# Fierykev/RayTraceBVH

Measured on AMD Instinct MI355X. Metric: Mrays/s primary+1-bounce (BASELINE.json's metric, on its config C5: 3840x2160, the 1/2/4/8-GPU config; the metric's @1080p config C3 is the line c3_1080p); BVH build Mtris/s under build, higher is better.
Workload: dtype f32; 1 GPU; C5: synthetic 10M tris (seed 0x5EED0005, box 100x100x50), 3840x2160, primary+1 bounce; width=3840, height=2160, bounces=1, triangles=10000000, parallelism=single GPU

## Files before the change

include/rtbvh.h:

```cpp
#ifndef RTBVH_H
#define RTBVH_H

#include <stddef.h>
#include <stdint.h>

#ifdef __cplusplus
extern "C" {
#endif

#define RTBVH_ABI_VERSION 8

typedef enum {
    RTBVH_OK = 0,
    RTBVH_ERR_INVALID_ARG = 1,
    RTBVH_ERR_HIP = 2,
    RTBVH_ERR_OOM = 3,
    RTBVH_ERR_NOT_READY = 4,
    RTBVH_ERR_STACK_OVERFLOW = 5,
    RTBVH_ERR_IO = 6,
    RTBVH_ERR_NO_DEVICE = 7,
    RTBVH_ERR_COMM = 8
} rtbvh_status;


// ... 7 lines not shown
    float ambient[4];
    float diffuse[4];
    float specular[4];
    float shininess;
    float optical_density;
    float alpha;
    uint32_t specularb;
    int32_t tex_num;
} rtbvh_material;

typedef struct {
    uint32_t parent, child_l, child_r, code;
    float bb_min[3], bb_max[3];
    uint32_t index;
} rtbvh_node;

typedef struct {
    float intensity;
    float origin[3], direction[3], inv_direction[3];
    float color[4];
} rtbvh_ray_present;

typedef struct {
    uint32_t width, height;
    const uint8_t* rgba8;
} rtbvh_texture;

enum {
    RTBVH_MORTON_CPUTESTS = 0,
    RTBVH_MORTON_HLSL = 1
};
enum {
    RTBVH_DELTA_CLZ64 = 0,
    RTBVH_DELTA_CPUTESTS = 1
};
enum {
    RTBVH_FLAG_TIMING = 1u << 0,
    RTBVH_FLAG_COUNT_VISITS = 1u << 1,
    RTBVH_FLAG_REFRACT_RECORDS = 1u << 2,
    RTBVH_FLAG_SORT_BOUNCE = 1u << 3,
    RTBVH_FLAG_NEAREST_FIRST = 1u << 4,
    RTBVH_FLAG_PACKET_PRIMARY = 1u << 5,
    RTBVH_FLAG_REFILL_BOUNCE = 1u << 6,
    RTBVH_FLAG_WIDE_BVH = 1u << 7,
    RTBVH_FLAG_AUTO_WALK = 1u << 8,
    RTBVH_FLAG_BINNED_PRIMARY = 1u << 9,
    RTBVH_FLAG_CERTIFIED = 1u << 10,
    RTBVH_FLAG_MULTI_KERNEL_BUILD = 1u << 16,
    RTBVH_FLAG_SPLIT_SHIFT = 17,
    RTBVH_FLAG_GRAPH = 1u << 20
};

typedef struct {
    int32_t device;
    uint32_t morton_mode;
    uint32_t delta_mode;
    uint32_t flags;
    float scene_bb_min[3];
    float scene_bb_max[3];
    void* stream;
    uint32_t stack_limit;
    uint32_t reserved;
} rtbvh_config;

typedef struct {
    uint32_t num_tris, num_nodes, width, height;
    uint64_t primary_rays, bounce_rays;
    uint64_t internal_visits[2], leaf_visits[2], hits[2];
    uint64_t textured_hits, stack_overflows;
    uint32_t timed_builds, timed_traces;
    float ms_build, ms_trace;
    float ms_stage[8];
    uint64_t trav_wave_steps, trav_mixed_steps, trav_active_lanes;
    uint64_t trav_max_steps, trav_steps_log2[32];
    uint64_t graph_captures;
    uint32_t walk_flags;
    uint32_t walk_state;
    uint64_t packet_steps[2];
    uint64_t cert_traces, redo_total;
    uint64_t bin_entries[2];
    uint64_t redo_rays[2];
    uint64_t trav_longest;
    uint64_t redo_deferred;
} rtbvh_stats;
typedef struct rtbvh_ctx rtbvh_ctx;

void rtbvh_config_default(rtbvh_config* cfg);
rtbvh_status rtbvh_create(const rtbvh_config* cfg, rtbvh_ctx** out);
void rtbvh_destroy(rtbvh_ctx* ctx);
const char* rtbvh_last_error(const rtbvh_ctx* ctx);
int rtbvh_abi_version(void);
uint32_t rtbvh_stats_size(void);

rtbvh_status rtbvh_set_scene(rtbvh_ctx* ctx, const rtbvh_vertex* verts, uint32_t nverts,
                             const uint32_t* indices, uint32_t nidx, const uint32_t* mat_idx,
                             const rtbvh_material* mats, uint32_t nmats,
                             const rtbvh_texture* textures, uint32_t ntex);
rtbvh_status rtbvh_set_camera(rtbvh_ctx* ctx, const float wvp[16], const float wv[16]);

rtbvh_status rtbvh_build(rtbvh_ctx* ctx);
rtbvh_status rtbvh_build_async(rtbvh_ctx* ctx);
rtbvh_status rtbvh_trace(rtbvh_ctx* ctx, uint32_t width, uint32_t height, uint32_t bounces);
rtbvh_status rtbvh_trace_async(rtbvh_ctx* ctx, uint32_t width, uint32_t height, uint32_t bounces);
rtbvh_status rtbvh_compute_bvh(rtbvh_ctx* ctx, uint32_t width, uint32_t height, uint32_t bounces);
rtbvh_status rtbvh_trace_band_async(rtbvh_ctx* ctx, uint32_t width, uint32_t height, uint32_t bounces,
                                    uint32_t rank, uint32_t nranks, float* dev_out, void* stream);
uint32_t rtbvh_band_rows(uint32_t height, uint32_t rank, uint32_t nranks);
uint32_t rtbvh_deal_bands(uint32_t height, uint32_t rank, uint32_t nranks, uint32_t root_share, uint32_t* bands,
                          uint32_t capacity);
uint32_t rtbvh_deal_rows(uint32_t height, uint32_t rank, uint32_t nranks, uint32_t root_share);
rtbvh_status rtbvh_set_band_deal(rtbvh_ctx* ctx, uint32_t root_share);
rtbvh_status rtbvh_verify_walk(rtbvh_ctx* ctx, uint32_t width, uint32_t height, uint32_t bounces,
                               uint64_t* differing_pixels);
rtbvh_status rtbvh_assemble_bands(rtbvh_ctx* ctx, uint32_t width, uint32_t height, uint32_t nranks,
                                  const float* dev_bands, uint32_t stride_rows, float* dev_frame, void* stream);

#define RTBVH_COMM_ID_BYTES 128
rtbvh_status rtbvh_comm_unique_id(uint8_t id[RTBVH_COMM_ID_BYTES]);
rtbvh_status rtbvh_comm_init(rtbvh_ctx* ctx, uint32_t nranks, uint32_t rank, const uint8_t id[RTBVH_COMM_ID_BYTES],
                             void** comm);
rtbvh_status rtbvh_comm_destroy(void* comm);
rtbvh_status rtbvh_trace_tiles(rtbvh_ctx* ctx, uint32_t width, uint32_t height, uint32_t bounces, uint32_t rank,
                               uint32_t nranks, void* comm);
rtbvh_status rtbvh_synchronize(rtbvh_ctx* ctx);

rtbvh_status rtbvh_update_vertices_async(rtbvh_ctx* ctx, const float* dev_positions, uint32_t pos_stride,
                                         const float* dev_normals, uint32_t nrm_stride,
                                         uint32_t first, uint32_t count, void* stream);
rtbvh_status rtbvh_update_vertices_host(rtbvh_ctx* ctx, const float* positions, uint32_t pos_stride,
                                        const float* normals, uint32_t nrm_stride,
                                        uint32_t first, uint32_t count);
rtbvh_status rtbvh_refit_async(rtbvh_ctx* ctx);
rtbvh_status rtbvh_refit(rtbvh_ctx* ctx);

typedef struct {
    float origin[3];
    float t_max;
    float direction[3];
    uint32_t reserved;
} rtbvh_ray;
typedef struct {
    float t, u, v;
    uint32_t tri;
} rtbvh_hit;
enum {
    RTBVH_QUERY_CLOSEST = 0,
    RTBVH_QUERY_ANY = 1u << 0,
    RTBVH_QUERY_SORT = 1u << 1,
    RTBVH_QUERY_COUNT = 1u << 2,
    RTBVH_QUERY_CERTIFIED = 1u << 8
};
rtbvh_status rtbvh_query_async(rtbvh_ctx* ctx, const rtbvh_ray* dev_rays, uint64_t n, rtbvh_hit* dev_hits,
                               uint32_t mode, void* stream);
rtbvh_status rtbvh_query_host(rtbvh_ctx* ctx, const rtbvh_ray* rays, uint64_t n, rtbvh_hit* hits, uint32_t mode);
rtbvh_status rtbvh_query_counts(rtbvh_ctx* ctx, uint64_t out[4]);
rtbvh_status rtbvh_query_walk_counts(rtbvh_ctx* ctx, uint64_t out[4]);


typedef struct {
    float point[3];
    float max_dist2;
} rtbvh_point;
typedef struct {
    float point[3];
    float dist2;
    float u, v;
// ... 75 lines not shown

typedef struct {
    float v0[3];
    uint32_t reserved0;
    float v1[3];
    uint32_t reserved1;
    float v2[3];
    uint32_t reserved2;
} rtbvh_tri;
enum {
    RTBVH_CROSS_SORT = 1u << 1,
    RTBVH_CROSS_COUNT = 1u << 2,
    RTBVH_CROSS_SIZES = 1u << 4,
    RTBVH_CROSS_FILL = 1u << 5
};
rtbvh_status rtbvh_cross_async(rtbvh_ctx* ctx, const rtbvh_tri* dev_tris, uint64_t n, uint64_t* dev_offsets,
                               uint32_t* dev_ids, uint64_t capacity, uint32_t mode, void* stream);
rtbvh_status rtbvh_cross_host(rtbvh_ctx* ctx, const rtbvh_tri* tris, uint64_t n, uint64_t* offsets, uint32_t* ids,
                              uint64_t capacity, uint32_t mode);
rtbvh_status rtbvh_cross_first_async(rtbvh_ctx* ctx, const rtbvh_tri* dev_tris, uint64_t n, uint32_t* dev_first,
                                     uint32_t mode, void* stream);
rtbvh_status rtbvh_cross_first_host(rtbvh_ctx* ctx, const rtbvh_tri* tris, uint64_t n, uint32_t* first,
                                    uint32_t mode);
rtbvh_status rtbvh_cross_counts(rtbvh_ctx* ctx, uint64_t out[4]);

typedef struct {
    float point_q[3];
    float dist2;
    float point_x[3];
    uint32_t tri;
} rtbvh_clearance;
enum {
    RTBVH_CLEARANCE_SORT = 1u << 1,
    RTBVH_CLEARANCE_COUNT = 1u << 2
};
rtbvh_status rtbvh_clearance_async(rtbvh_ctx* ctx, const rtbvh_tri* dev_tris, uint64_t n, float max_dist2,
                                   rtbvh_clearance* dev_out, uint32_t mode, void* stream);
rtbvh_status rtbvh_clearance_host(rtbvh_ctx* ctx, const rtbvh_tri* tris, uint64_t n, float max_dist2,
                                  rtbvh_clearance* out, uint32_t mode);
rtbvh_status rtbvh_clearance_counts(rtbvh_ctx* ctx, uint64_t out[4]);

typedef struct {
    float lo[3];
    uint32_t reserved0;
    float hi[3];
    uint32_t reserved1;
} rtbvh_box;
enum {
    RTBVH_OVERLAP_SORT = 1u << 1,
    RTBVH_OVERLAP_COUNT = 1u << 2,
    RTBVH_OVERLAP_TRIANGLE = 1u << 3,
    RTBVH_OVERLAP_SIZES = 1u << 4,
    RTBVH_OVERLAP_FILL = 1u << 5
};
rtbvh_status rtbvh_overlap_async(rtbvh_ctx* ctx, const rtbvh_box* dev_boxes, uint64_t n, uint64_t* dev_offsets,
                                 uint32_t* dev_ids, uint64_t capacity, uint32_t mode, void* stream);
rtbvh_status rtbvh_overlap_host(rtbvh_ctx* ctx, const rtbvh_box* boxes, uint64_t n, uint64_t* offsets,
                                uint32_t* ids, uint64_t capacity, uint32_t mode);
rtbvh_status rtbvh_overlap_counts(rtbvh_ctx* ctx, uint64_t out[4]);

typedef struct {
    float point[3]; float dist2;
    float u, v; uint32_t tri;
    uint32_t flags;
} rtbvh_signed;
enum { RTBVH_SIGNED_SORT = 1u << 1, RTBVH_SIGNED_COUNT = 1u << 2,
       RTBVH_SIGNED_VOTE3 = 1u << 3,
       RTBVH_SIGNED_INSIDE_ONLY = 1u << 4
        };
rtbvh_status rtbvh_signed_async(rtbvh_ctx* ctx, const rtbvh_point* dev_points, uint64_t n, rtbvh_signed* dev_out,
                                uint32_t mode, void* stream);
rtbvh_status rtbvh_signed_host(rtbvh_ctx* ctx, const rtbvh_point* points, uint64_t n, rtbvh_signed* out,
                               uint32_t mode);
rtbvh_status rtbvh_signed_counts(rtbvh_ctx* ctx, uint64_t out[4]);

rtbvh_status rtbvh_read_framebuffer(rtbvh_ctx* ctx, float* rgba);
rtbvh_status rtbvh_read_intensity(rtbvh_ctx* ctx, float* intensity);
rtbvh_status rtbvh_present(rtbvh_ctx* ctx, uint8_t* rgba8);
rtbvh_status rtbvh_save_bmp(const char* path, const uint8_t* rgba8, uint32_t width, uint32_t height);
const float* rtbvh_framebuffer_device(rtbvh_ctx* ctx);
rtbvh_status rtbvh_read_bvh(rtbvh_ctx* ctx, rtbvh_node* out, uint32_t capacity);
rtbvh_status rtbvh_read_wide(rtbvh_ctx* ctx, uint32_t* records, uint64_t capacity);
rtbvh_status rtbvh_read_qnodes(rtbvh_ctx* ctx, uint32_t* nodes, uint64_t capacity);
rtbvh_status rtbvh_read_morton(rtbvh_ctx* ctx, uint32_t* codes);
rtbvh_status rtbvh_read_sorted(rtbvh_ctx* ctx, uint32_t* sorted_codes, uint32_t* tri_ids);
rtbvh_status rtbvh_read_rays(rtbvh_ctx* ctx, rtbvh_ray_present* reflect_out, rtbvh_ray_present* refract_out);
rtbvh_status rtbvh_get_stats(rtbvh_ctx* ctx, rtbvh_stats* out);
rtbvh_status rtbvh_reset_stats(rtbvh_ctx* ctx);
rtbvh_status rtbvh_set_flags(rtbvh_ctx* ctx, uint32_t flags);
uint64_t rtbvh_bin_builds(rtbvh_ctx* ctx);
uint32_t rtbvh_bin_sets(rtbvh_ctx* ctx);

rtbvh_status rtbvh_sort_pairs_async(rtbvh_ctx* ctx, uint32_t* keys_in, uint32_t* vals_in,
                                    uint32_t* keys_out, uint32_t* vals_out, uint32_t n,
                                    uint32_t key_bits);
rtbvh_status rtbvh_sort_pairs_host(rtbvh_ctx* ctx, const uint32_t* keys, const uint32_t* vals,
                                   uint32_t* keys_out, uint32_t* vals_out, uint32_t n, uint32_t key_bits);
rtbvh_status rtbvh_build_from_codes(rtbvh_ctx* ctx, const uint32_t* sorted_codes,
                                    const float* leaf_boxes, uint32_t n, rtbvh_node* out);

rtbvh_status rtbvh_texture_load_bmp(const char* path, rtbvh_texture* out);
rtbvh_status rtbvh_texture_load_jpeg(const char* path, rtbvh_texture* out);
rtbvh_status rtbvh_texture_decode_jpeg(const uint8_t* data, size_t size, rtbvh_texture* out);
rtbvh_status rtbvh_texture_load(const char* path, rtbvh_texture* out);
void rtbvh_texture_free(rtbvh_texture* tex);
void rtbvh_srgb_table(float out[256]);
typedef struct rtbvh_scene rtbvh_scene;
rtbvh_status rtbvh_scene_load_obj(const char* path, rtbvh_scene** out);
rtbvh_status rtbvh_scene_synthetic(uint64_t seed, uint32_t ntris, const float half_extent[3],
                                   rtbvh_scene** out);
void rtbvh_scene_free(rtbvh_scene* s);
uint32_t rtbvh_scene_num_vertices(const rtbvh_scene* s);
uint32_t rtbvh_scene_num_indices(const rtbvh_scene* s);
uint32_t rtbvh_scene_num_materials(const rtbvh_scene* s);
uint32_t rtbvh_scene_num_textures(const rtbvh_scene* s);
const rtbvh_vertex* rtbvh_scene_vertices(const rtbvh_scene* s);
const uint32_t* rtbvh_scene_indices(const rtbvh_scene* s);
const uint32_t* rtbvh_scene_mat_indices(const rtbvh_scene* s);
const rtbvh_material* rtbvh_scene_materials(const rtbvh_scene* s);
const char* rtbvh_scene_texture_path(const rtbvh_scene* s, uint32_t k);
rtbvh_status rtbvh_set_scene_obj(rtbvh_ctx* ctx, const rtbvh_scene* s, const rtbvh_texture* textures,
                                 uint32_t ntex);
void rtbvh_camera_reference(uint32_t width, uint32_t height, float wvp[16], float wv[16]);
void rtbvh_camera_look(const float eye[3], uint32_t width, uint32_t height, float wvp[16], float wv[16]);
void rtbvh_camera_orbit(float eye[3], uint32_t key);

#ifdef __cplusplus
}
#endif
#endif
```

raytracebvh_amd/_lib.py:

```python
from __future__ import annotations

import ctypes
import os

import numpy as np

HERE = os.path.dirname(os.path.abspath(__file__))
LIB_PATH = os.environ.get("RTBVH_LIB") or os.path.join(HERE, "librtbvh.so")

OK, ERR_INVALID_ARG, ERR_HIP, ERR_OOM, ERR_NOT_READY, ERR_STACK_OVERFLOW, ERR_IO, ERR_NO_DEVICE = range(8)
MORTON_CPUTESTS, MORTON_HLSL = 0, 1
DELTA_CLZ64, DELTA_CPUTESTS = 0, 1
FLAG_TIMING, FLAG_COUNT_VISITS, FLAG_REFRACT_RECORDS, FLAG_SORT_BOUNCE, FLAG_NEAREST_FIRST = 1, 2, 4, 8, 16
FLAG_PACKET_PRIMARY = 1 << 5
FLAG_REFILL_BOUNCE = 1 << 6
FLAG_WIDE_BVH = 1 << 7
FLAG_BINNED_PRIMARY = 1 << 9
FLAG_CERTIFIED = 1 << 10
FLAG_MULTI_KERNEL_BUILD = 1 << 16
FLAG_AUTO_WALK = 1 << 8
FLAG_SPLIT_SHIFT = 17
FLAG_GRAPH = 1 << 20

EXPORTS = [
    "rtbvh_config_default", "rtbvh_create", "rtbvh_destroy", "rtbvh_last_error", "rtbvh_abi_version", "rtbvh_stats_size",
    "rtbvh_set_scene", "rtbvh_set_camera", "rtbvh_build", "rtbvh_build_async", "rtbvh_trace",
    "rtbvh_trace_async", "rtbvh_compute_bvh", "rtbvh_trace_band_async", "rtbvh_band_rows", "rtbvh_verify_walk",
    "rtbvh_deal_bands", "rtbvh_deal_rows", "rtbvh_set_band_deal",
    "rtbvh_synchronize", "rtbvh_read_framebuffer", "rtbvh_read_intensity", "rtbvh_framebuffer_device",
    "rtbvh_read_bvh", "rtbvh_read_wide", "rtbvh_read_qnodes", "rtbvh_read_morton", "rtbvh_read_sorted", "rtbvh_read_rays", "rtbvh_get_stats",
    "rtbvh_reset_stats", "rtbvh_set_flags", "rtbvh_bin_builds", "rtbvh_bin_sets",
    "rtbvh_sort_pairs_async", "rtbvh_sort_pairs_host", "rtbvh_build_from_codes", "rtbvh_scene_load_obj",
    "rtbvh_scene_synthetic", "rtbvh_scene_free", "rtbvh_scene_num_vertices", "rtbvh_scene_num_indices",
    "rtbvh_scene_num_materials", "rtbvh_scene_num_textures", "rtbvh_scene_vertices", "rtbvh_scene_indices",
    "rtbvh_scene_mat_indices", "rtbvh_scene_materials", "rtbvh_scene_texture_path", "rtbvh_set_scene_obj",
    "rtbvh_camera_reference", "rtbvh_camera_look", "rtbvh_camera_orbit", "rtbvh_texture_load_bmp", "rtbvh_texture_load_jpeg", "rtbvh_texture_decode_jpeg",
    "rtbvh_texture_load", "rtbvh_texture_free", "rtbvh_srgb_table",
    "rtbvh_present", "rtbvh_save_bmp", "rtbvh_assemble_bands", "rtbvh_comm_unique_id", "rtbvh_comm_init",
    "rtbvh_comm_destroy", "rtbvh_trace_tiles",
    "rtbvh_query_async", "rtbvh_query_host", "rtbvh_query_counts", "rtbvh_query_walk_counts",
    "rtbvh_nearest_async", "rtbvh_nearest_host", "rtbvh_nearest_counts",
    "rtbvh_within_async", "rtbvh_within_host", "rtbvh_within_counts",
    "rtbvh_knn_async", "rtbvh_knn_host", "rtbvh_knn_counts",
    "rtbvh_allhits_async", "rtbvh_allhits_host", "rtbvh_allhits_counts",
    "rtbvh_overlap_async", "rtbvh_overlap_host", "rtbvh_overlap_counts",
    "rtbvh_signed_async", "rtbvh_signed_host", "rtbvh_signed_counts",
    "rtbvh_khits_async", "rtbvh_khits_host", "rtbvh_khits_counts",
    "rtbvh_collide_async", "rtbvh_collide_host", "rtbvh_collide_counts",
    "rtbvh_cross_async", "rtbvh_cross_host", "rtbvh_cross_first_async", "rtbvh_cross_first_host", "rtbvh_cross_counts",
    "rtbvh_clearance_async", "rtbvh_clearance_host", "rtbvh_clearance_counts",
    "rtbvh_update_vertices_async", "rtbvh_update_vertices_host", "rtbvh_refit_async", "rtbvh_refit",
]
COMM_ID_BYTES = 128

NODE_DTYPE = np.dtype([("parent", "<u4"), ("child_l", "<u4"), ("child_r", "<u4"), ("code", "<u4"),
                       ("bb_min", "<f4", (3,)), ("bb_max", "<f4", (3,)), ("index", "<u4")])
MATERIAL_DTYPE = np.dtype([("ambient", "<f4", (4,)), ("diffuse", "<f4", (4,)), ("specular", "<f4", (4,)),
                           ("shininess", "<f4"), ("optical_density", "<f4"), ("alpha", "<f4"),
                           ("specularb", "<u4"), ("tex_num", "<i4")])
assert NODE_DTYPE.itemsize == 44 and MATERIAL_DTYPE.itemsize == 68
RAY_DTYPE = np.dtype([("origin", "<f4", (3,)), ("t_max", "<f4"), ("direction", "<f4", (3,)), ("reserved", "<u4")])
HIT_DTYPE = np.dtype([("t", "<f4"), ("u", "<f4"), ("v", "<f4"), ("tri", "<u4")])
assert RAY_DTYPE.itemsize == 32 and HIT_DTYPE.itemsize == 16
QUERY_CLOSEST, QUERY_ANY, QUERY_SORT, QUERY_COUNT = 0, 1, 2, 4
QUERY_CERTIFIED = 1 << 8
POINT_DTYPE = np.dtype([("point", "<f4", (3,)), ("max_dist2", "<f4")])
NEAREST_DTYPE = np.dtype([("point", "<f4", (3,)), ("dist2", "<f4"), ("u", "<f4"), ("v", "<f4"), ("tri", "<u4"),
                          ("reserved", "<u4")])
assert POINT_DTYPE.itemsize == 16 and NEAREST_DTYPE.itemsize == 32
NEAREST_SORT, NEAREST_COUNT = 2, 4
PAIR_DTYPE = np.dtype([("tri", "<u4"), ("dist2", "<f4")])
assert PAIR_DTYPE.itemsize == 8
WITHIN_SORT, WITHIN_COUNT, WITHIN_SIZES, WITHIN_FILL = 2, 4, 16, 32
KNN_SORT, KNN_COUNT = 2, 4
KNN_MAX_K = 32
ALLHITS_SORT, ALLHITS_COUNT, ALLHITS_BY_T, ALLHITS_SIZES, ALLHITS_FILL = 2, 4, 8, 16, 32
BOX_DTYPE = np.dtype([("lo", "<f4", (3,)), ("reserved0", "<u4"), ("hi", "<f4", (3,)), ("reserved1", "<u4")])
assert BOX_DTYPE.itemsize == 32
OVERLAP_SORT, OVERLAP_COUNT, OVERLAP_TRIANGLE, OVERLAP_SIZES, OVERLAP_FILL = 2, 4, 8, 16, 32
SIGNED_DTYPE = np.dtype([("point", "<f4", (3,)), ("dist2", "<f4"), ("u", "<f4"), ("v", "<f4"), ("tri", "<u4"),
                         ("flags", "<u4")])
assert SIGNED_DTYPE.itemsize == 32
SIGNED_SORT, SIGNED_COUNT, SIGNED_VOTE3, SIGNED_INSIDE_ONLY = 2, 4, 8, 16
KHITS_SORT, KHITS_COUNT = 2, 4
KHITS_MAX_K = 16
COLLIDE_COUNT, COLLIDE_TRIANGLE, COLLIDE_SIZES, COLLIDE_FILL, COLLIDE_SYMMETRIC = 4, 8, 16, 32, 64
TRI_DTYPE = np.dtype([("v0", "<f4", (3,)), ("reserved0", "<u4"), ("v1", "<f4", (3,)), ("reserved1", "<u4"),
                      ("v2", "<f4", (3,)), ("reserved2", "<u4")])
assert TRI_DTYPE.itemsize == 48
CROSS_SORT, CROSS_COUNT, CROSS_SIZES, CROSS_FILL = 2, 4, 16, 32
CLEARANCE_DTYPE = np.dtype([("point_q", "<f4", (3,)), ("dist2", "<f4"), ("point_x", "<f4", (3,)), ("tri", "<u4")])
assert CLEARANCE_DTYPE.itemsize == 32
CLEARANCE_SORT, CLEARANCE_COUNT = 2, 4


class Config(ctypes.Structure):
    _fields_ = [("device", ctypes.c_int32), ("morton_mode", ctypes.c_uint32), ("delta_mode", ctypes.c_uint32),
                ("flags", ctypes.c_uint32), ("scene_bb_min", ctypes.c_float * 3),
                ("scene_bb_max", ctypes.c_float * 3), ("stream", ctypes.c_void_p),
                ("stack_limit", ctypes.c_uint32), ("reserved", ctypes.c_uint32)]


class Ray(ctypes.Structure):
    _fields_ = [("origin", ctypes.c_float * 3), ("t_max", ctypes.c_float), ("direction", ctypes.c_float * 3),
                ("reserved", ctypes.c_uint32)]


class Hit(ctypes.Structure):
    _fields_ = [("t", ctypes.c_float), ("u", ctypes.c_float), ("v", ctypes.c_float), ("tri", ctypes.c_uint32)]


class Point(ctypes.Structure):
    _fields_ = [("point", ctypes.c_float * 3), ("max_dist2", ctypes.c_float)]


class Nearest(ctypes.Structure):
    _fields_ = [("point", ctypes.c_float * 3), ("dist2", ctypes.c_float), ("u", ctypes.c_float), ("v", ctypes.c_float),
                ("tri", ctypes.c_uint32), ("reserved", ctypes.c_uint32)]


class Texture(ctypes.Structure):
    _fields_ = [("width", ctypes.c_uint32), ("height", ctypes.c_uint32), ("rgba8", ctypes.c_void_p)]


class Stats(ctypes.Structure):
    _fields_ = [("num_tris", ctypes.c_uint32), ("num_nodes", ctypes.c_uint32), ("width", ctypes.c_uint32),
                ("height", ctypes.c_uint32), ("primary_rays", ctypes.c_uint64), ("bounce_rays", ctypes.c_uint64),
                ("internal_visits", ctypes.c_uint64 * 2), ("leaf_visits", ctypes.c_uint64 * 2),
                ("hits", ctypes.c_uint64 * 2), ("textured_hits", ctypes.c_uint64),
                ("stack_overflows", ctypes.c_uint64), ("timed_builds", ctypes.c_uint32),
                ("timed_traces", ctypes.c_uint32), ("ms_build", ctypes.c_float), ("ms_trace", ctypes.c_float),
                ("ms_stage", ctypes.c_float * 8), ("trav_wave_steps", ctypes.c_uint64),
                ("trav_mixed_steps", ctypes.c_uint64), ("trav_active_lanes", ctypes.c_uint64),
                ("trav_max_steps", ctypes.c_uint64), ("trav_steps_log2", ctypes.c_uint64 * 32),
                ("graph_captures", ctypes.c_uint64), ("walk_flags", ctypes.c_uint32),
                ("walk_state", ctypes.c_uint32), ("packet_steps", ctypes.c_uint64 * 2),
                ("cert_traces", ctypes.c_uint64), ("redo_total", ctypes.c_uint64),
                ("bin_entries", ctypes.c_uint64 * 2), ("redo_rays", ctypes.c_uint64 * 2),
                ("trav_longest", ctypes.c_uint64), ("redo_deferred", ctypes.c_uint64)]

    def as_dict(self) -> dict:
        d = {}
        for k, _ in self._fields_:
            v = getattr(self, k)
            d[k] = list(v) if hasattr(v, "__len__") else v
        return d


class RtbvhError(RuntimeError):
    def __init__(self, status: int, msg: str):
        super().__init__(f"rtbvh status {status}: {msg}")
        self.status = status


_lib = None


def lib() -> ctypes.CDLL:
    global _lib
    if _lib is not None:
        return _lib
    if not os.path.exists(LIB_PATH):
        raise ImportError(f"{LIB_PATH} is not built: run `python -c 'import __graft_entry__ as g; g.build()'` "
                          "(there is no CPU fallback for the HIP path)")
    try:
        import torch
    except ImportError:
        pass
    L = ctypes.CDLL(LIB_PATH)
    vp, u32, u64, i32 = ctypes.c_void_p, ctypes.c_uint32, ctypes.c_uint64, ctypes.c_int
    sig = {
        "rtbvh_config_default": (None, [ctypes.POINTER(Config)]),
        "rtbvh_create": (i32, [ctypes.POINTER(Config), ctypes.POINTER(vp)]),
        "rtbvh_destroy": (None, [vp]),
        "rtbvh_last_error": (ctypes.c_char_p, [vp]),
        "rtbvh_abi_version": (i32, []),
        "rtbvh_stats_size": (ctypes.c_uint32, []),
        "rtbvh_set_scene": (i32, [vp, vp, u32, vp, u32, vp, vp, u32, vp, u32]),
        "rtbvh_set_camera": (i32, [vp, vp, vp]),
        "rtbvh_build": (i32, [vp]),
        "rtbvh_build_async": (i32, [vp]),
        "rtbvh_trace": (i32, [vp, u32, u32, u32]),
        "rtbvh_trace_async": (i32, [vp, u32, u32, u32]),
        "rtbvh_compute_bvh": (i32, [vp, u32, u32, u32]),
        "rtbvh_trace_band_async": (i32, [vp, u32, u32, u32, u32, u32, vp, vp]),
        "rtbvh_band_rows": (u32, [u32, u32, u32]),
        "rtbvh_deal_bands": (u32, [u32, u32, u32, u32, vp, u32]),
        "rtbvh_deal_rows": (u32, [u32, u32, u32, u32]),
        "rtbvh_set_band_deal": (i32, [vp, u32]),
        "rtbvh_verify_walk": (i32, [vp, u32, u32, u32, ctypes.POINTER(u64)]),
        "rtbvh_assemble_bands": (i32, [vp, u32, u32, u32, vp, u32, vp, vp]),
        "rtbvh_comm_unique_id": (i32, [vp]),
        "rtbvh_comm_init": (i32, [vp, u32, u32, vp, ctypes.POINTER(vp)]),
        "rtbvh_comm_destroy": (i32, [vp]),
        "rtbvh_trace_tiles": (i32, [vp, u32, u32, u32, u32, u32, vp]),
        "rtbvh_synchronize": (i32, [vp]),
        "rtbvh_read_framebuffer": (i32, [vp, vp]),
        "rtbvh_read_intensity": (i32, [vp, vp]),
        "rtbvh_framebuffer_device": (vp, [vp]),
        "rtbvh_read_bvh": (i32, [vp, vp, u32]),
        "rtbvh_read_morton": (i32, [vp, vp]),
        "rtbvh_read_wide": (i32, [vp, vp, ctypes.c_uint64]),
        "rtbvh_read_qnodes": (i32, [vp, vp, ctypes.c_uint64]),
        "rtbvh_read_sorted": (i32, [vp, vp, vp]),
        "rtbvh_read_rays": (i32, [vp, vp, vp]),
        "rtbvh_get_stats": (i32, [vp, ctypes.POINTER(Stats)]),
        "rtbvh_reset_stats": (i32, [vp]),
        "rtbvh_set_flags": (i32, [vp, u32]),
        "rtbvh_bin_builds": (u64, [vp]),
        "rtbvh_bin_sets": (u32, [vp]),
        "rtbvh_sort_pairs_async": (i32, [vp, vp, vp, vp, vp, u32, u32]),
        "rtbvh_sort_pairs_host": (i32, [vp, vp, vp, vp, vp, u32, u32]),
        "rtbvh_build_from_codes": (i32, [vp, vp, vp, u32, vp]),
        "rtbvh_scene_load_obj": (i32, [ctypes.c_char_p, ctypes.POINTER(vp)]),
        "rtbvh_scene_synthetic": (i32, [u64, u32, vp, ctypes.POINTER(vp)]),
        "rtbvh_scene_free": (None, [vp]),
        "rtbvh_scene_num_vertices": (u32, [vp]),
        "rtbvh_scene_num_indices": (u32, [vp]),
        "rtbvh_scene_num_materials": (u32, [vp]),
        "rtbvh_scene_num_textures": (u32, [vp]),
        "rtbvh_scene_vertices": (vp, [vp]),
        "rtbvh_scene_indices": (vp, [vp]),
        "rtbvh_scene_mat_indices": (vp, [vp]),
        "rtbvh_scene_materials": (vp, [vp]),
        "rtbvh_scene_texture_path": (ctypes.c_char_p, [vp, u32]),
        "rtbvh_set_scene_obj": (i32, [vp, vp, vp, u32]),
        "rtbvh_camera_reference": (None, [u32, u32, vp, vp]),
        "rtbvh_camera_look": (None, [vp, u32, u32, vp, vp]),
        "rtbvh_camera_orbit": (None, [vp, u32]),
        "rtbvh_texture_load_bmp": (i32, [ctypes.c_char_p, vp]),
        "rtbvh_texture_load_jpeg": (i32, [ctypes.c_char_p, vp]),
        "rtbvh_texture_decode_jpeg": (i32, [vp, ctypes.c_size_t, vp]),
        "rtbvh_texture_load": (i32, [ctypes.c_char_p, vp]),
        "rtbvh_texture_free": (None, [vp]),
        "rtbvh_srgb_table": (None, [vp]),
        "rtbvh_present": (i32, [vp, vp]),
        "rtbvh_save_bmp": (i32, [ctypes.c_char_p, vp, u32, u32]),
        "rtbvh_query_async": (i32, [vp, vp, u64, vp, u32, vp]),
        "rtbvh_query_host": (i32, [vp, vp, u64, vp, u32]),
        "rtbvh_query_counts": (i32, [vp, vp]),
        "rtbvh_query_walk_counts": (i32, [vp, vp]),
        "rtbvh_nearest_async": (i32, [vp, vp, u64, vp, u32, vp]),
        "rtbvh_nearest_host": (i32, [vp, vp, u64, vp, u32]),
        "rtbvh_nearest_counts": (i32, [vp, vp]),
        "rtbvh_within_async": (i32, [vp, vp, u64, vp, vp, u64, u32, vp]),
        "rtbvh_within_host": (i32, [vp, vp, u64, vp, vp, u64, u32]),
        "rtbvh_within_counts": (i32, [vp, vp]),
        "rtbvh_knn_async": (i32, [vp, vp, u64, u32, vp, u32, vp]),
        "rtbvh_knn_host": (i32, [vp, vp, u64, u32, vp, u32]),
        "rtbvh_knn_counts": (i32, [vp, vp]),
        "rtbvh_signed_async": (i32, [vp, vp, u64, vp, u32, vp]),
        "rtbvh_signed_host": (i32, [vp, vp, u64, vp, u32]),
        "rtbvh_signed_counts": (i32, [vp, vp]),
        "rtbvh_khits_async": (i32, [vp, vp, u64, u32, vp, u32, vp]),
        "rtbvh_khits_host": (i32, [vp, vp, u64, u32, vp, u32]),
        "rtbvh_khits_counts": (i32, [vp, vp]),
        "rtbvh_allhits_async": (i32, [vp, vp, u64, vp, vp, u64, u32, vp]),
        "rtbvh_allhits_host": (i32, [vp, vp, u64, vp, vp, u64, u32]),
        "rtbvh_allhits_counts": (i32, [vp, vp]),
        "rtbvh_overlap_async": (i32, [vp, vp, u64, vp, vp, u64, u32, vp]),
        "rtbvh_overlap_host": (i32, [vp, vp, u64, vp, vp, u64, u32]),
        "rtbvh_overlap_counts": (i32, [vp, vp]),
        "rtbvh_collide_async": (i32, [vp, vp, vp, u64, u32, vp]),
        "rtbvh_collide_host": (i32, [vp, vp, vp, u64, u32]),
        "rtbvh_collide_counts": (i32, [vp, vp]),
        "rtbvh_cross_async": (i32, [vp, vp, u64, vp, vp, u64, u32, vp]),
        "rtbvh_cross_host": (i32, [vp, vp, u64, vp, vp, u64, u32]),
        "rtbvh_cross_first_async": (i32, [vp, vp, u64, vp, u32, vp]),
        "rtbvh_cross_first_host": (i32, [vp, vp, u64, vp, u32]),
        "rtbvh_cross_counts": (i32, [vp, vp]),
        "rtbvh_clearance_async": (i32, [vp, vp, u64, ctypes.c_float, vp, u32, vp]),
        "rtbvh_clearance_host": (i32, [vp, vp, u64, ctypes.c_float, vp, u32]),
        "rtbvh_clearance_counts": (i32, [vp, vp]),
        "rtbvh_update_vertices_async": (i32, [vp, vp, u32, vp, u32, u32, u32, vp]),
        "rtbvh_update_vertices_host": (i32, [vp, vp, u32, vp, u32, u32, u32]),
        "rtbvh_refit_async": (i32, [vp]),
        "rtbvh_refit": (i32, [vp]),
    }
    for name, (res, args) in sig.items():
        f = getattr(L, name)
        f.restype = res
        f.argtypes = args
    _lib = L
    return L


# ... 12 lines not shown
```

raytracebvh_amd/csrc/api.hip:

```cpp
#include <dlfcn.h>
#include <rccl/rccl.h>

#include <algorithm>
#include <cstdio>
#include <cstring>
#include <deque>
#include <new>
#include <string>
#include <type_traits>
#include <utility>
#include <vector>

#include "../../include/rtbvh.h"
#include "rtbvh_internal.h"

using namespace rtbvh;

#ifndef RTBVH_MAXSPLIT
#define RTBVH_MAXSPLIT 4
#endif

template <typename H, void (*Del)(H)>
struct Owner {
    H h{};
    Owner() = default;
    Owner(Owner&& o) noexcept : h(o.h) { o.h = H{}; }
    Owner& operator=(Owner&& o) noexcept {
        std::swap(h, o.h);
        return *this;
    }
    ~Owner() { reset(); }
    void reset() {
        if (h) Del(h);
        h = H{};
    }
    H* out() {
        reset();
        return &h;
    }
    operator H() const { return h; }
};
template <typename T> void del_device(T* p) { (void)hipFree((void*)p); }
template <typename T> void del_pinned(T* p) { (void)hipHostFree((void*)p); }
inline void del_event(hipEvent_t e) { (void)hipEventDestroy(e); }
inline void del_stream(hipStream_t s) {
    (void)hipStreamSynchronize(s);
    (void)hipStreamDestroy(s);
}
template <typename T>
struct DevBuf : Owner<T*, del_device<T>> {
    hipError_t alloc(size_t count) { return hipMalloc((void**)this->out(), (count ? count : 1) * sizeof(T)); }
};
template <typename T>
struct Pinned : Owner<T*, del_pinned<T>> {
    hipError_t alloc(size_t count) {
        return hipHostMalloc((void**)this->out(), count * sizeof(T), hipHostMallocDefault);
    }
};
using Event = Owner<hipEvent_t, del_event>;
using Stream = Owner<hipStream_t, del_stream>;
template <typename T>
struct Grown {
    DevBuf<T> buf;
    size_t cap = 0;
    bool has(size_t n) const { return n == 0 || (n <= cap && buf); }
    hipError_t reserve(size_t n) {
        if (has(n)) return hipSuccess;
        const hipError_t e = buf.alloc(n);
        if (e != hipSuccess) buf.h = nullptr;
        cap = e == hipSuccess ? n : 0;
        return e;
    }
    void reset() {
        buf.reset();
        cap = 0;
    }
    operator T*() const { return buf.h; }
};

enum Form : uint32_t { RECORDS = 1, NBOX = 2, PSEUDO = 4, QNODES = 8 };
struct Tree {
    bool built = false;
    bool clz64 = false;
    Form wrote = RECORDS;
    uint32_t valid = 0;
};

struct PbKey {
    uint64_t build = 0;
    uint32_t W = 0, H = 0, rows = 0, rank = 0, nranks = 0, T = 0, ntx = 0, nty = 0;
    uint32_t share = 0;
    const uint32_t* deal = nullptr;
    bool operator==(const PbKey& o) const {
        return build == o.build && W == o.W && H == o.H && rows == o.rows && rank == o.rank &&
               nranks == o.nranks && T == o.T && ntx == o.ntx && nty == o.nty && share == o.share &&
               deal == o.deal;
    }
};
struct PbBufs {
    DevBuf<uint32_t> off, cur, sums;
    DevBuf<uint4> bins;
    uint32_t cap_T = 0, cap_tiles = 0, cap_bins = 0;
    Grown<uint32_t> list;
    PbKey key;
    bool valid = false;
    Event filled;
    uint32_t readers = 0;
};

struct TraceSet {
    Stream chain;
    Event join;
    hipStream_t caller = nullptr;
    Event done;
    bool busy = false;
    DevBuf<RayQ> q[2];
    DevBuf<float2> hit;
    Grown<uint32_t> redo, defer;
    PbBufs pb;
    Grown<unsigned long long> pbkeys;
    uint32_t* qcount = nullptr;
    uint32_t* next = nullptr;
    unsigned long long* counters = nullptr;
    unsigned long long* ovf = nullptr;
};

struct LastTrace {
    bool traced = false;
    uint32_t W = 0, H = 0, bounces = 0, rank = 0, nranks = 1;
    uint32_t nsplit = 1;
    uint32_t slot = 0;
    size_t rec_P = 0;
    uint32_t walk = 0;
    uint32_t walk_state = 0;
    bool cert = false;
    bool frame_here = false;
    bool intensity_here = false;
};

struct rtbvh_ctx {
    rtbvh_config cfg{};
    Stream own_stream, side;
    static constexpr uint32_t MAXSPLIT = RTBVH_MAXSPLIT;
    TraceSet sets[MAXSPLIT];
    hipStream_t stream = nullptr;
    std::string err;

    uint32_t V = 0, T = 0, nmat = 0;
    DevBuf<float4> d_opos;
    DevBuf<float> d_verts;
    DevBuf<uint32_t> d_idx, d_matidx;
    DevBuf<Mat> d_mats;
    float wvp[16], wv[16];
    DevBuf<float> d_cam;
    bool cam_dirty = false;
    bool have_scene = false, have_camera = false;
    Tree tree;
    Event ev_update;
    bool update_pending = false;
    bool stale = false;

    uint32_t cap_T = 0;
    DevBuf<uint32_t> d_codes, d_ids, d_ka, d_va, d_kb, d_vb, d_sort_scratch;
    DevBuf<float4> d_tclip, d_leaf;
    Grown<float4> d_band;
    DevBuf<Inner> d_inner;
    DevBuf<uint4> d_topo;
    DevBuf<Inner> d_rec;
    DevBuf<QNode> d_qnode;
    DevBuf<uint4> d_lfp;
    DevBuf<uint32_t> d_texels;
    DevBuf<uint4> d_texinfo;
    DevBuf<float> d_srgb;
    uint32_t ntex = 0;
    Grown<float> d_refl_rec;
    Grown<float> d_refr_rec;
    DevBuf<uint32_t> d_pleaf, d_pint, d_cnt;
    DevBuf<uint32_t> d_xlist, d_xcnt;
    DevBuf<uint32_t> d_qlate;
    DevBuf<unsigned long long> d_ovf;
    Pinned<unsigned long long> h_ovf;
    unsigned long long ovf_seen = 0;
    DevBuf<float> d_bounds, d_rootbox, d_zpart;
    Event ev_leaf, ev_prim;
    DevBuf<float> d_nbox;
    bool tail_pending = false;
    bool leaf_pending = false;
    SortResult sorted{nullptr, nullptr};

    size_t cap_P = 0;
    DevBuf<float4> d_color;
    DevBuf<float> d_intensity;
    DevBuf<uint32_t> d_bkin, d_bvin, d_bka, d_bva, d_bkb, d_bvb, d_bscratch;
    DevBuf<uint32_t> d_qcount;
    DevBuf<uint32_t> d_next;
    DevBuf<unsigned long long> d_counters;
    size_t cap_split = 0;
    Event ev_fork;
    uint64_t bins_epoch = 1;
    uint64_t bin_builds = 0;
    bool knob_bins_reuse = true;
    LastTrace last;

    static constexpr int RING = 32;
    Event evb[RING][6];
    Event evt[RING][5];
    bool evt_trav[RING] = {};
    uint32_t n_builds = 0, n_traces = 0;
    Event ev_built;
    bool slots_used = false;
    hipGraph_t graph = nullptr;
    hipGraphExec_t graph_exec = nullptr;
    uint64_t graph_key[5] = {};
    bool capturing = false;
    uint64_t graph_captures = 0;
    LastTrace graph_trace;
    Tree graph_tree;
    uint64_t cert_traces = 0;
    uint64_t small_key = 0;
    uint32_t small_flags = 0;
    bool small_packet = false;
    Event ev_small[2];
    uint32_t knob_bounce_blocks = 0;
    bool knob_overlap = false, knob_side_priority = true, knob_keep_records = false, knob_no_early_shade = false,
         knob_no_small_tiles = false;
    uint32_t root_share = 16;
    struct DealTab {
        uint32_t H, nranks, share;
        DevBuf<uint32_t> d;
        std::vector<uint32_t> off;
        Pinned<uint32_t> h;
        Event ready;
    };
    std::deque<DealTab> deals;
    static constexpr size_t MAX_DEALS = 8;
    DevBuf<uint32_t> d_qscratch;
    Grown<uint32_t> d_qsort;
    Grown<uint32_t> d_qsort_scratch;
    Grown<uint32_t> d_qredo;
    Grown<unsigned long long> d_qscan;
    Grown<uint32_t> d_qorder;
    Event ev_query;
    bool query_busy = false;
    bool query_ovf = false;
    bool query_counted = false;
    uint64_t query_fallback = 0;
    bool nearest_counted = false;
    bool within_counted = false;
    bool allhits_counted = false;
    bool overlap_counted = false;
    bool knn_counted = false;
    bool signed_counted = false;
    bool khits_counted = false;
    bool collide_counted = false;
    bool cross_counted = false;
    bool clearance_counted = false;
};

namespace {

std::string g_create_error;

rtbvh_status fail(rtbvh_ctx* c, rtbvh_status st, const std::string& msg) {
    if (c) c->err = msg;
    else g_create_error = msg;
    return st;
}

#define HIPC(ctx, expr)                                                                          \
    do {                                                                                         \
        hipError_t _e = (expr);                                                                  \
        if (_e != hipSuccess)                                                                    \
            return fail(ctx, _e == hipErrorOutOfMemory ? RTBVH_ERR_OOM : RTBVH_ERR_HIP,          \
                        std::string(#expr) + ": " + hipGetErrorString(_e));                      \
    } while (0)
#define TRY(expr)                                      \
    do {                                               \
        if (rtbvh_status _st = (expr)) return _st;     \
    } while (0)

void drop_graph(rtbvh_ctx* c) {
    if (c->graph_exec) (void)hipGraphExecDestroy(c->graph_exec);
    if (c->graph) (void)hipGraphDestroy(c->graph);
    c->graph_exec = nullptr;
    c->graph = nullptr;
}

void reset_tree(rtbvh_ctx* c) {
    c->tree = Tree{};
    c->stale = false;
    c->bins_epoch++;
    c->tail_pending = c->leaf_pending = false;
}

rtbvh_status check_launch(rtbvh_ctx* c, const char* what) {
    hipError_t e = hipGetLastError();
    if (e != hipSuccess) return fail(c, RTBVH_ERR_HIP, std::string(what) + ": " + hipGetErrorString(e));
    return RTBVH_OK;
}

rtbvh_status drain_slots(rtbvh_ctx* c) {
    for (TraceSet& t : c->sets)
        if (t.busy) HIPC(c, hipEventSynchronize(t.done));
    return RTBVH_OK;
}
rtbvh_status sync_all(rtbvh_ctx* c) {
    HIPC(c, hipStreamSynchronize(c->stream));
    TRY(drain_slots(c));
    if (c->query_busy) HIPC(c, hipEventSynchronize(c->ev_query));
    if (c->update_pending) HIPC(c, hipEventSynchronize(c->ev_update));
    return RTBVH_OK;
}

rtbvh_status wait_slots(rtbvh_ctx* c, hipStream_t s) {
    for (TraceSet& t : c->sets)
        if (t.busy) {
            HIPC(c, hipStreamWaitEvent(s, t.done, 0));
            t.busy = false;
        }
    return RTBVH_OK;
}

rtbvh_status wait_queries(rtbvh_ctx* c, hipStream_t s) {
    if (c->query_busy) {
        HIPC(c, hipStreamWaitEvent(s, c->ev_query, 0));
        c->query_busy = false;
    }
    return RTBVH_OK;
}

rtbvh_status wait_update(rtbvh_ctx* c, hipStream_t s) {
    if (c->update_pending) {
        HIPC(c, hipStreamWaitEvent(s, c->ev_update, 0));
        c->update_pending = false;
    }
    return RTBVH_OK;
}
rtbvh_status fail_stale(rtbvh_ctx* c, const char* what) {
    return fail(c, RTBVH_ERR_NOT_READY,
                std::string(what) + ": the vertices were updated after the last build -- the tree is not of this "
                                    "geometry until rtbvh_build, rtbvh_refit or rtbvh_compute_bvh");
}

rtbvh_status order_after_context(rtbvh_ctx* c, hipStream_t s) {
    if (!c->capturing) HIPC(c, hipEventRecord(c->ev_built, c->stream));
    if (s != c->stream) HIPC(c, hipStreamWaitEvent(s, c->ev_built, 0));
    return RTBVH_OK;
}

rtbvh_status ensure_build_capacity(rtbvh_ctx* c, uint32_t T) {
    if (T <= c->cap_T && c->d_codes) return RTBVH_OK;
    drop_graph(c);
    reset_tree(c);
    const size_t n = T, ni = T > 1 ? T - 1 : 1;
    HIPC(c, c->d_codes.alloc(n));
    HIPC(c, c->d_ids.alloc(n));
    HIPC(c, c->d_ka.alloc(n));
    HIPC(c, c->d_va.alloc(n));
    HIPC(c, c->d_kb.alloc(n));
    HIPC(c, c->d_vb.alloc(n));
    HIPC(c, c->d_sort_scratch.alloc(sort_scratch_words(T)));
    HIPC(c, c->d_tclip.alloc(TCS * n));
    HIPC(c, c->d_leaf.alloc(4 * n));
    HIPC(c, c->d_inner.alloc(ni));
    HIPC(c, c->d_topo.alloc(ni));
    HIPC(c, c->d_rec.alloc(2 * (size_t)n - 1));
    HIPC(c, c->d_nbox.alloc(6 * (size_t)ni));
    HIPC(c, c->d_qnode.alloc(2 * (size_t)n - 1));
    HIPC(c, c->d_lfp.alloc(n));
    HIPC(c, c->d_pleaf.alloc(n));
    HIPC(c, c->d_pint.alloc(ni));
    HIPC(c, c->d_cnt.alloc(ni));
    HIPC(c, c->d_xlist.alloc(n));
    HIPC(c, c->d_qlate.alloc(n + 1));
    HIPC(c, c->d_xcnt.alloc(refit_blocks(T)));
    HIPC(c, c->d_zpart.alloc(ZPART * (size_t)refit_blocks(T)));
    HIPC(c, c->d_bounds.alloc(BOUNDS_WORDS));
    HIPC(c, c->d_rootbox.alloc(ROOTBOX_WORDS));
    c->cap_T = T;
    return RTBVH_OK;
}

rtbvh_status ensure_trace_capacity(rtbvh_ctx* c, size_t P) {
    if (P <= c->cap_P && c->d_color) return RTBVH_OK;
    drop_graph(c);
    HIPC(c, c->d_color.alloc(P));
    HIPC(c, c->d_intensity.alloc(P));
    HIPC(c, c->sets[0].q[0].alloc(P));
    HIPC(c, c->sets[0].q[1].alloc(P));
    HIPC(c, c->d_bkin.alloc(P));
    HIPC(c, c->d_bvin.alloc(P));
    HIPC(c, c->d_bka.alloc(P));
    HIPC(c, c->d_bva.alloc(P));
    HIPC(c, c->d_bkb.alloc(P));
    HIPC(c, c->d_bvb.alloc(P));
    HIPC(c, c->d_bscratch.alloc(sort_scratch_words((uint32_t)P)));
    HIPC(c, c->sets[0].hit.alloc(P));
    if (!c->d_qcount) HIPC(c, c->d_qcount.alloc(32 * rtbvh_ctx::MAXSPLIT));
    if (!c->d_next) HIPC(c, c->d_next.alloc((size_t)NEXT_WORDS * rtbvh_ctx::MAXSPLIT));
    if (!c->d_counters) HIPC(c, c->d_counters.alloc(64 * rtbvh_ctx::MAXSPLIT));
    for (uint32_t b = 0; b < rtbvh_ctx::MAXSPLIT; b++) {
        c->sets[b].qcount = c->d_qcount + 32 * b;
        c->sets[b].next = c->d_next + (size_t)NEXT_WORDS * b;
        c->sets[b].counters = c->d_counters + 64 * b;
    }
    c->cap_P = P;
    return RTBVH_OK;
}

uint32_t trace_split(const rtbvh_ctx* c) {
    const uint32_t v = (c->cfg.flags >> RTBVH_FLAG_SPLIT_SHIFT) & 7u;
    if (v) return v < rtbvh_ctx::MAXSPLIT ? v : rtbvh_ctx::MAXSPLIT;
    return 1;
}

rtbvh_status ensure_split_capacity(rtbvh_ctx* c, uint32_t nsets, size_t rays) {
    if (nsets < 2) return RTBVH_OK;
    const bool grow = rays > c->cap_split;
    if (grow) {
        drop_graph(c);
        TRY(drain_slots(c));
        c->cap_split = rays;
        for (uint32_t g = nsets; g < rtbvh_ctx::MAXSPLIT; g++) {
            TraceSet& t = c->sets[g];
            t.q[0].reset(); t.q[1].reset(); t.hit.reset();
        }
    }
    for (uint32_t g = 1; g < nsets; g++) {
        TraceSet& t = c->sets[g];
        if (!t.chain) HIPC(c, hipStreamCreateWithFlags(t.chain.out(), hipStreamNonBlocking));
        if (!t.join) HIPC(c, hipEventCreateWithFlags(t.join.out(), hipEventDisableTiming));
        if (!c->ev_fork) HIPC(c, hipEventCreateWithFlags(c->ev_fork.out(), hipEventDisableTiming));
        if (t.q[0] && !grow) continue;
        HIPC(c, t.q[0].alloc(c->cap_split));
        HIPC(c, t.q[1].alloc(c->cap_split));
        HIPC(c, t.hit.alloc(c->cap_split));
// ... 248 lines not shown
    std::string err;
    ncclResult_t (*GetUniqueId)(ncclUniqueId*) = nullptr;
    ncclResult_t (*CommInitRank)(ncclComm_t*, int, ncclUniqueId, int) = nullptr;
    ncclResult_t (*CommDestroy)(ncclComm_t) = nullptr;
    ncclResult_t (*Send)(const void*, size_t, ncclDataType_t, int, ncclComm_t, hipStream_t) = nullptr;
    ncclResult_t (*Recv)(void*, size_t, ncclDataType_t, int, ncclComm_t, hipStream_t) = nullptr;
    ncclResult_t (*GroupStart)() = nullptr;
    ncclResult_t (*GroupEnd)() = nullptr;
    const char* (*GetErrorString)(ncclResult_t) = nullptr;
};
const Rccl& rccl() {
    static const Rccl lib = [] {
        Rccl r;
        void* h = dlopen("librccl.so.1", RTLD_NOW | RTLD_GLOBAL);
        if (!h) {
            const char* e = dlerror();
            r.err = std::string("RCCL not available: ") + (e ? e : "dlopen(librccl.so.1) failed");
            return r;
        }
        bool all = true;
        auto sym = [&](auto& f, const char* name) {
            f = reinterpret_cast<std::remove_reference_t<decltype(f)>>(dlsym(h, name));
            if (!f) all = false;
        };
        sym(r.GetUniqueId, "ncclGetUniqueId");
        sym(r.CommInitRank, "ncclCommInitRank");
        sym(r.CommDestroy, "ncclCommDestroy");
        sym(r.Send, "ncclSend");
        sym(r.Recv, "ncclRecv");
        sym(r.GroupStart, "ncclGroupStart");
        sym(r.GroupEnd, "ncclGroupEnd");
        sym(r.GetErrorString, "ncclGetErrorString");
        r.ok = all;
        if (!all) r.err = "RCCL: librccl.so.1 lacks a required symbol";
        return r;
    }();
    return lib;
}

rtbvh_status sync_camera(rtbvh_ctx* c, hipStream_t s) {
    if (!c->cam_dirty) return RTBVH_OK;
    TRY(wait_slots(c, c->stream));
    launch_set_camera(c->wvp, c->wv, c->d_cam, c->stream);
    HIPC(c, hipGetLastError());
    c->cam_dirty = false;
    return order_after_context(c, s);
}

rtbvh_status before_tree_write(rtbvh_ctx* c, hipStream_t s) {
    TRY(wait_slots(c, s));
    TRY(wait_queries(c, s));
    TRY(wait_update(c, s));
    TRY(sync_camera(c, s));
    c->bins_epoch++;
    return RTBVH_OK;
}

struct TailGuard {
    rtbvh_ctx* c;
    bool pending;
    void run() {
        if (pending) launch_refit_tail(build_args(c), c->stream);
        pending = false;
    }
    ~TailGuard() { run(); }
};

struct WalkPlan {
    hipStream_t s;
    uint32_t slot, bounces;
    bool cert;
    bool leaf_pending;
    bool count, timing, records;
    Walks wk;
    PrimaryKind pkind;
    Form nodes;
    uint32_t P, rows;
    uint32_t nsplit, Pg;
    uint32_t tblocks;
    uint32_t ntx, nty;
    bool inflight, fuse_tail, overlap, small_tiles, early_shade;
    uint32_t bset;
    bool fill_bins;
};

WalkPlan plan_walks(const rtbvh_ctx* c, const TraceArgs& a, uint32_t bounces, hipStream_t s, uint32_t slot,
                    uint32_t flags, bool cert, bool timed, bool tail_pending, bool leaf_pending) {
    WalkPlan p{s, slot, bounces, cert, leaf_pending};
    p.bset = slot;
    p.count = (c->cfg.flags & RTBVH_FLAG_COUNT_VISITS) != 0;
    p.timing = timed && (c->cfg.flags & RTBVH_FLAG_TIMING) != 0 && s == c->stream && !c->capturing;
    p.wk = choose_walks(flags);
    p.records = (flags & RTBVH_FLAG_REFRACT_RECORDS) != 0;
    p.P = a.W * deal_rows(a.H, a.rank, a.nranks, c->root_share);
    p.rows = p.P / a.W;
#ifndef RTBVH_BOUNCE_GRID
#define RTBVH_BOUNCE_GRID (256 * BOUNCE_WAVES)
#endif
    p.inflight = slot != 0;
    for (uint32_t k = 1; k < rtbvh_ctx::MAXSPLIT && !p.inflight && !c->capturing; k++)
        p.inflight = c->sets[k].busy && hipEventQuery(c->sets[k].done) == hipErrorNotReady;
    p.tblocks = p.P < (1u << 22) ? (!p.inflight ? 1536 : p.P < (3u << 20) ? 512 : 1024) : RTBVH_BOUNCE_GRID;
    if (c->knob_bounce_blocks) p.tblocks = c->knob_bounce_blocks;
    const bool binned = p.wk.primary == PrimaryKind::BINNED;
    p.pkind = binned && (a.W > 32768u || a.H > 32768u)
                  ? (cert ? PrimaryKind::LANE_REFERENCE : PrimaryKind::PACKET_WIDE)
                  : p.wk.primary;
    p.nsplit = trace_split(c);
    if (p.wk.sort || a.my_bands < p.nsplit || slot || c->slots_used || binned) p.nsplit = 1;
    p.Pg = p.nsplit == 1 ? p.P : a.W * 8 * ((a.my_bands + p.nsplit - 1) / p.nsplit);
    p.nodes = cert ? NBOX : RECORDS;
    p.fuse_tail = tail_pending && p.pkind == PrimaryKind::BINNED && s == c->stream && slot == 0 && p.rows > 0 &&
                  (c->tree.valid & p.nodes);
    p.overlap = p.pkind == PrimaryKind::BINNED && leaf_pending && s == c->stream && slot == 0 && p.nsplit == 1;
    p.ntx = pb_tiles_x(a.W);
    p.nty = pb_tiles_y(p.rows);
    p.small_tiles = !p.inflight && !c->knob_no_small_tiles && (size_t)a.W * p.rows < (3u << 19);
    p.early_shade = cert && !p.inflight && !c->knob_no_early_shade;
    return p;
}

rtbvh_status prepare_walks(rtbvh_ctx* c, WalkPlan& p, TraceArgs& a, const rtbvh_ctx::DealTab* deal, TailGuard& tail) {
    hipStream_t s = p.s;
    TraceSet& mine = c->sets[p.slot];
    const size_t P = p.P;
    if (p.records) {
        if (!(c->d_refl_rec.has(14 * P) && c->d_refr_rec.has(14 * P))) {
            drop_graph(c);
            HIPC(c, c->d_refl_rec.reserve(14 * P));
            HIPC(c, c->d_refr_rec.reserve(14 * P));
        }
        a.refl_rec = c->d_refl_rec;
        a.refr_rec = c->d_refr_rec;
    }
    if (!p.fuse_tail && tail.pending) {
        tail.run();
        TRY(order_after_context(c, s));
    }
    TRY(ensure_form(c, p.nodes, s));
    a.nb = p.cert;
    TRY(ensure_split_capacity(c, p.slot ? p.slot + 1 : p.nsplit, p.Pg));
    if (p.bounces > 0 && p.wk.refill && p.wk.bounce == BounceWalk::WIDE_QUANTIZED) TRY(ensure_form(c, QNODES, s));
    if (p.pkind == PrimaryKind::PACKET_REFERENCE || p.pkind == PrimaryKind::PACKET_NEAREST ||
        p.pkind == PrimaryKind::PACKET_WIDE)
        TRY(ensure_form(c, PSEUDO, s));
    if (p.cert && p.bounces > 0 && !mine.defer.has(P)) {
        drop_graph(c);
        HIPC(c, mine.defer.reserve(P));
        if (hipMemsetAsync(mine.defer, 0, sizeof(uint32_t) * P, c->stream) != hipSuccess) {
            mine.defer.reset();
            return fail(c, RTBVH_ERR_HIP, "clearing the deferred-ray list failed");
        }
        TRY(order_after_context(c, s));
    }
    if (p.cert && !mine.redo.has(P)) {
        drop_graph(c);
        HIPC(c, mine.redo.reserve(P));
    }
    if (p.pkind != PrimaryKind::BINNED || p.rows == 0) return RTBVH_OK;
    const size_t px = (size_t)a.W * p.rows;
    if (pb_keys_used() && !mine.pbkeys.has(px)) {
        drop_graph(c);
        HIPC(c, mine.pbkeys.reserve(px));
    }
    const PbKey key{c->bins_epoch, a.W, a.H, p.rows, a.rank, a.nranks, c->T, p.ntx, p.nty,
                    a.nranks > 1 ? c->root_share : 16u, deal ? deal->d.h : nullptr};
    const int found = p.fuse_tail || p.leaf_pending ? -1 : find_bins(c, key);
    if (found >= 0) {
        p.bset = (uint32_t)found;
        PbBufs& pb = c->sets[p.bset].pb;
        if (p.bset != p.slot) HIPC(c, hipStreamWaitEvent(s, pb.filled, 0));
        pb.readers |= 1u << p.slot;
        return RTBVH_OK;
    }
    p.fill_bins = true;
    PbBufs& pb = mine.pb;
    TRY(ensure_pb_capacity(c, pb, c->T, p.ntx * p.nty));
    if (a.nranks > 1 && !pb.list.has(pb_list_words(c->T))) {
        drop_graph(c);
        HIPC(c, pb.list.reserve(pb_list_words(c->T)));
    }
    for (uint32_t k = 0; k < rtbvh_ctx::MAXSPLIT && !c->capturing; k++) {
        if (k == p.slot || !(pb.readers & 1u << k)) continue;
        if (k == 0) TRY(order_after_context(c, s));
        else if (c->sets[k].done) HIPC(c, hipStreamWaitEvent(s, c->sets[k].done, 0));
    }
    pb.readers = 1u << p.slot;
    pb.valid = false;
    pb.key = key;
    return RTBVH_OK;
}

rtbvh_status launch_walks(rtbvh_ctx* c, const WalkPlan& p, const TraceArgs& a, TailGuard& tail) {
    hipStream_t s = p.s;
    TraceSet& mine = c->sets[p.slot];
    const uint32_t bounces = p.bounces, nsplit = p.nsplit;
    const bool count = p.count, cert = p.cert, refill = p.wk.refill;
    Event* ev = c->evt[c->n_traces % rtbvh_ctx::RING];
    ZeroList z{};
    z.ptr[0] = reinterpret_cast<uint32_t*>(mine.counters);
    z.words[0] = 64 * 2;
    z.ptr[1] = mine.qcount;
    z.words[1] = 32 * nsplit;
    if (refill && bounces) {
        z.ptr[2] = mine.next;
        z.words[2] = (size_t)NEXT_WORDS * nsplit;
    }
    if (p.fill_bins) {
        z.ptr[3] = mine.pb.off;
        z.words[3] = (size_t)p.ntx * p.nty * PB_NZ + 1;
        if (a.nranks > 1) {
            z.ptr[4] = mine.pb.list;
            z.words[4] = (size_t)PB_LISTS * PB_LIST_STRIDE;
        }
    }
    hipStream_t sp = s;
    if (p.overlap) {
        sp = c->side;
        HIPC(c, hipStreamWaitEvent(sp, c->ev_leaf, 0));
    }
    launch_zero(z, sp);
    if (p.timing) HIPC(c, hipEventRecord(ev[0], sp));
    if (nsplit > 1) HIPC(c, hipEventRecord(c->ev_fork, s));
    for (uint32_t g = 0; g < nsplit; g++) {
        TraceSet& set = c->sets[p.slot + g];
// ... 17 lines not shown
                    c->bin_builds++;
                    if (c->knob_bins_reuse && !c->capturing) {
                        if (!pbb.filled) HIPC(c, hipEventCreateWithFlags(pbb.filled.out(), hipEventDisableTiming));
                        HIPC(c, hipEventRecord(pbb.filled, sp));
                        pbb.valid = true;
                    }
                }
                launch_pb_raster(ag, pb, p.rows, q[0], &qc[0], count, bounces > 0, sp, cert ? &rd : nullptr,
                                 p.small_tiles);
                if (p.fuse_tail) tail.pending = false;
            }
            if (p.overlap) {
                HIPC(c, hipEventRecord(c->ev_prim, sp));
                HIPC(c, hipStreamWaitEvent(sg, c->ev_prim, 0));
            }
            if (p.rows) launch_pb_gate(ag, pb, q[0], &qc[0], count, bounces > 0, sg, cert);
        } else
            launch_primary(ag, q[0], &qc[0], count, bounces > 0, p.pkind, sg);
        if (tg) HIPC(c, hipEventRecord(ev[1], sg));
        for (uint32_t b = 0; b < bounces; b++) {
            const uint32_t* perm = nullptr;
            if (p.wk.sort) {
                launch_bounce_keys(q[b & 1], &qc[b], c->d_rootbox, p.P, c->d_bkin, c->d_bvin, sg);
                perm = radix_sort_pairs(c->d_bkin, c->d_bvin, c->d_bka, c->d_bva, c->d_bkb, c->d_bvb, p.P, 30,
                                        c->d_bscratch, sg).vals;
            }
            if (refill) {
                if (tg && b == 0) HIPC(c, hipEventRecord(ev[3], sg));
                uint32_t* nxb = set.next + (size_t)NEXT_SEGS * NEXT_STRIDE * b;
                const BounceShade es{q[(b + 1) & 1], &qc[b + 1], b + 1 < bounces, mine.redo, &qc[17 + b], p.Pg};
                launch_bounce_traverse(ag, q[b & 1], &qc[b], perm, count, p.wk.bounce, set.hit, nxb, p.tblocks, sg, cert,
                                       mine.defer, p.early_shade ? &es : nullptr);
                if (tg && b == 0) HIPC(c, hipEventRecord(ev[4], sg));
                const Redo rd{mine.redo, &qc[17 + b], mine.defer, nxb};
                launch_bounce_shade(ag, q[b & 1], &qc[b], set.hit, q[(b + 1) & 1], &qc[b + 1], count, b + 1 < bounces,
                                    p.Pg, sg, cert ? &rd : nullptr);
            } else
                launch_bounce(ag, q[b & 1], &qc[b], perm, q[(b + 1) & 1], &qc[b + 1], count, b + 1 < bounces,
                              p.wk.nearest, sg);
        }
        if (g) {
            HIPC(c, hipEventRecord(set.join, sg));
            HIPC(c, hipStreamWaitEvent(s, set.join, 0));
        }
    }
    HIPC(c, hipMemcpyAsync(mine.ovf, c->d_ovf, sizeof(unsigned long long), hipMemcpyDeviceToHost, s));
    if (p.timing) {
        HIPC(c, hipEventRecord(ev[2], s));
        c->evt_trav[c->n_traces % rtbvh_ctx::RING] = refill && bounces > 0;
        c->n_traces++;
    }
    return RTBVH_OK;
}

rtbvh_status enqueue_walks(rtbvh_ctx* c, uint32_t W, uint32_t H, uint32_t bounces, uint32_t rank, uint32_t nranks,
                           float4* color, float* inten, hipStream_t s, uint32_t slot, uint32_t flags, bool timed,
                           uint32_t walk_state, bool cert = false) {
    const bool leaf_pending = c->leaf_pending;
    c->leaf_pending = false;
    TailGuard tail{c, c->tail_pending};
    c->tail_pending = false;
    if (!c->tree.built) return fail(c, RTBVH_ERR_NOT_READY, "trace before build");
    if (c->stale) return fail_stale(c, "trace");
    if (W == 0 || H == 0 || nranks == 0 || rank >= nranks || bounces > 14)
        return fail(c, RTBVH_ERR_INVALID_ARG, "bad trace dimensions");
    TRY(ensure_trace_capacity(c, (size_t)W * H));
    if (!color) color = c->d_color;
    TraceArgs a = trace_args(c, W, H, rank, nranks, color, inten);
    const rtbvh_ctx::DealTab* deal = nullptr;
    TRY(get_deal(c, H, nranks, &deal, s));
    if (deal) {
        a.my_bands = deal->off[rank + 1] - deal->off[rank];
        a.band_list = deal->d + deal->off[rank];
        a.band_slots = deal->d + (H + 7) / 8;
    }
    a.counters = c->sets[slot].counters;
    if ((flags & RTBVH_FLAG_REFRACT_RECORDS) && slot)
        return fail(c, RTBVH_ERR_INVALID_ARG, "ray records are traced on the context stream only");
    WalkPlan p = plan_walks(c, a, bounces, s, slot, flags, cert, timed, tail.pending, leaf_pending);
    TRY(prepare_walks(c, p, a, deal, tail));
    TRY(launch_walks(c, p, a, tail));
    const bool frame_here = color == c->d_color && nranks == 1;
    c->last = LastTrace{true, W, H, bounces, rank, nranks, p.nsplit, slot, p.records ? p.P : 0, flags & WALK_FLAGS,
                        walk_state, cert, frame_here, frame_here && inten != nullptr};
    return check_launch(c, "trace kernels");
}

struct TracePlan {
    uint32_t flags;
    bool cert;
    uint32_t state;
};
TracePlan plan_trace(const rtbvh_ctx* c, uint32_t f) {
    if (!(f & (RTBVH_FLAG_AUTO_WALK | RTBVH_FLAG_CERTIFIED))) return TracePlan{f, false, 0};
    const uint32_t ref = f & ~WALK_FLAGS;
    const bool limited = c->cfg.stack_limit != 0 && c->cfg.stack_limit < (uint32_t)STACK_SIZE;
    const bool want = (f & RTBVH_FLAG_CERTIFIED) || auto_checked(c);
    if (!want || !c->tree.clz64 || limited) return TracePlan{ref, false, 0};
    return TracePlan{ref | RTBVH_FLAG_NEAREST_FIRST | RTBVH_FLAG_REFILL_BOUNCE | RTBVH_FLAG_WIDE_BVH |
                         RTBVH_FLAG_BINNED_PRIMARY,
                     true, 2};
}

rtbvh_status enqueue_trace(rtbvh_ctx* c, uint32_t W, uint32_t H, uint32_t bounces, uint32_t rank, uint32_t nranks,
                           float4* color, float* inten, hipStream_t s, uint32_t slot = 0) {
    if (!c->tree.built) return fail(c, RTBVH_ERR_NOT_READY, "trace before build");
    if (c->stale) return fail_stale(c, "trace");
    TRY(sync_camera(c, s));
    TracePlan p = plan_trace(c, c->cfg.flags);
    if (p.cert && !c->capturing) c->cert_traces++;
    const uint32_t f = c->cfg.flags;
    const bool limited = c->cfg.stack_limit != 0 && c->cfg.stack_limit < (uint32_t)STACK_SIZE;
    if ((f & RTBVH_FLAG_AUTO_WALK) && !p.cert && c->tree.clz64 && !limited) {
        const uint64_t key = (uint64_t)W << 48 | (uint64_t)H << 32 | c->T;
        const uint32_t fw = f & (WALK_FLAGS | RTBVH_FLAG_AUTO_WALK | RTBVH_FLAG_CERTIFIED | RTBVH_FLAG_SORT_BOUNCE);
        if ((c->small_key != key || c->small_flags != fw) && !c->capturing && s == c->stream && slot == 0 &&
            nranks == 1) {
            Event* ev = c->ev_small;
            for (int k = 0; k < 2; k++)
                if (!ev[k]) HIPC(c, hipEventCreate(ev[k].out()));
            float best[2] = {INFINITY, INFINITY};
            for (int round = 0; round < 2; round++)
                for (int k = 0; k < 2; k++) {
                    HIPC(c, hipEventRecord(ev[0], s));
                    TRY(enqueue_walks(c, W, H, 0, 0, 1, color, inten, s, 0,
                                      p.flags | (k ? RTBVH_FLAG_PACKET_PRIMARY : 0u), false, p.state));
                    HIPC(c, hipEventRecord(ev[1], s));
                    HIPC(c, hipEventSynchronize(ev[1]));
                    float ms = 0.f;
                    HIPC(c, hipEventElapsedTime(&ms, ev[0], ev[1]));
                    best[k] = std::min(best[k], ms);
                }
            c->small_packet = best[1] < 0.95f * best[0];
            c->small_key = key;
            c->small_flags = fw;
        }
        if (c->small_key == key && c->small_flags == fw && c->small_packet) p.flags |= RTBVH_FLAG_PACKET_PRIMARY;
    }
    return enqueue_walks(c, W, H, bounces, rank, nranks, color, inten, s, slot, p.flags, true, p.state, p.cert);
}

}

extern "C" {

int rtbvh_abi_version(void) { return RTBVH_ABI_VERSION; }
uint32_t rtbvh_stats_size(void) { return (uint32_t)sizeof(rtbvh_stats); }

void rtbvh_config_default(rtbvh_config* cfg) {
    if (!cfg) return;
    memset(cfg, 0, sizeof(*cfg));
    cfg->device = 0;
    cfg->morton_mode = RTBVH_MORTON_CPUTESTS;
    cfg->delta_mode = RTBVH_DELTA_CLZ64;
    for (int k = 0; k < 3; k++) {
        cfg->scene_bb_min[k] = -700.f;
        cfg->scene_bb_max[k] = 700.f;
    }
}

rtbvh_status rtbvh_create(const rtbvh_config* cfg, rtbvh_ctx** out) {
    if (!out) return fail(nullptr, RTBVH_ERR_INVALID_ARG, "out is NULL");
    *out = nullptr;
    rtbvh_ctx* c = new (std::nothrow) rtbvh_ctx();
    if (!c) return fail(nullptr, RTBVH_ERR_OOM, "host allocation failed");
    if (cfg) c->cfg = *cfg;
    else rtbvh_config_default(&c->cfg);
    if (c->cfg.morton_mode > 1 || c->cfg.delta_mode > 1 || c->cfg.reserved != 0) {
        delete c;
        return fail(nullptr, RTBVH_ERR_INVALID_ARG, "bad morton/delta mode");
    }
    int ndev = 0;
    if (hipGetDeviceCount(&ndev) != hipSuccess || ndev <= 0) {
        delete c;
        return fail(nullptr, RTBVH_ERR_NO_DEVICE, "no HIP device");
    }
    if (c->cfg.device < 0 || c->cfg.device >= ndev || hipSetDevice(c->cfg.device) != hipSuccess) {
        delete c;
        return fail(nullptr, RTBVH_ERR_NO_DEVICE, "bad device ordinal");
    }
    if (c->cfg.stream) {
        c->stream = (hipStream_t)c->cfg.stream;
    } else {
        if (hipStreamCreateWithFlags(c->own_stream.out(), hipStreamNonBlocking) != hipSuccess) {
            delete c;
            return fail(nullptr, RTBVH_ERR_HIP, "hipStreamCreate failed");
        }
        c->stream = c->own_stream;
    }
    bool ev_ok = true;
    for (auto& row : c->evb)
        for (auto& e : row) ev_ok = ev_ok && hipEventCreate(e.out()) == hipSuccess;
    for (auto& row : c->evt)
        for (auto& e : row) ev_ok = ev_ok && hipEventCreate(e.out()) == hipSuccess;
    if (!ev_ok) {
        rtbvh_destroy(c);
        return fail(nullptr, RTBVH_ERR_HIP, "hipEventCreate failed");
    }
    if (hipEventCreateWithFlags(c->ev_built.out(), hipEventDisableTiming) != hipSuccess) {
        rtbvh_destroy(c);
        return fail(nullptr, RTBVH_ERR_HIP, "hipEventCreate failed");
    }
    if (c->d_ovf.alloc(1) != hipSuccess || hipMemset(c->d_ovf, 0, sizeof(unsigned long long)) != hipSuccess ||
        c->h_ovf.alloc(rtbvh_ctx::MAXSPLIT) != hipSuccess) {
        rtbvh_destroy(c);
        return fail(nullptr, RTBVH_ERR_OOM, "overflow counter allocation failed");
    }
    memset(c->h_ovf, 0, sizeof(unsigned long long) * rtbvh_ctx::MAXSPLIT);
    for (uint32_t b = 0; b < rtbvh_ctx::MAXSPLIT; b++) c->sets[b].ovf = c->h_ovf + b;
    if (c->d_cam.alloc(32) != hipSuccess ||
        hipMemset(c->d_cam, 0, 32 * sizeof(float)) != hipSuccess) {
        rtbvh_destroy(c);
        return fail(nullptr, RTBVH_ERR_OOM, "camera buffer allocation failed");
    }
    if (const char* e = getenv("RTBVH_BOUNCE_BLOCKS")) c->knob_bounce_blocks = (uint32_t)std::max(0, atoi(e));
    if (const char* e = getenv("RTBVH_OVERLAP")) c->knob_overlap = atoi(e) != 0;
    if (const char* e = getenv("RTBVH_SIDE_PRIORITY")) c->knob_side_priority = atoi(e) != 0;
    if (const char* e = getenv("RTBVH_KEEP_RECORDS")) c->knob_keep_records = atoi(e) != 0;
    if (const char* e = getenv("RTBVH_EARLY_SHADE")) c->knob_no_early_shade = atoi(e) == 0;
    if (const char* e = getenv("RTBVH_PB_SMALL_TILES")) c->knob_no_small_tiles = atoi(e) == 0;
    if (const char* e = getenv("RTBVH_BINS_REUSE")) c->knob_bins_reuse = atoi(e) != 0;
    *out = c;
    return RTBVH_OK;
}

void rtbvh_destroy(rtbvh_ctx* c) {
    if (!c) return;
    (void)hipSetDevice(c->cfg.device);
    (void)sync_all(c);
    drop_graph(c);
    delete c;
}

const char* rtbvh_last_error(const rtbvh_ctx* c) { return c ? c->err.c_str() : g_create_error.c_str(); }

rtbvh_status rtbvh_set_scene(rtbvh_ctx* c, const rtbvh_vertex* verts, uint32_t nverts, const uint32_t* indices,
                             uint32_t nidx, const uint32_t* mat_idx, const rtbvh_material* mats, uint32_t nmats,
                             const rtbvh_texture* textures, uint32_t ntex) {
    if (!c) return RTBVH_ERR_INVALID_ARG;
    drop_graph(c);
    if (ntex && !textures) return fail(c, RTBVH_ERR_INVALID_ARG, "set_scene: ntex > 0 without textures");
    for (uint32_t k = 0; k < ntex; k++)
        if (textures[k].width == 0 || textures[k].height == 0 || !textures[k].rgba8)
            return fail(c, RTBVH_ERR_INVALID_ARG, "set_scene: empty texture");
    if (!verts || !indices || !mat_idx || !mats || nverts == 0 || nidx == 0 || nidx % 3 != 0 || nmats == 0)
        return fail(c, RTBVH_ERR_INVALID_ARG, "set_scene: empty or ragged input");
    const uint32_t T = nidx / 3;
    if (T >= (1u << 30)) return fail(c, RTBVH_ERR_INVALID_ARG, "set_scene: too many triangles");
    for (uint32_t i = 0; i < nidx; i++)
        if (indices[i] >= nverts) return fail(c, RTBVH_ERR_INVALID_ARG, "set_scene: index out of range");
    for (uint32_t t = 0; t < T; t++)
        if (mat_idx[t] >= nmats) return fail(c, RTBVH_ERR_INVALID_ARG, "set_scene: material index out of range");
    HIPC(c, hipSetDevice(c->cfg.device));
    TRY(sync_all(c));
    c->query_busy = false;
    reset_tree(c);
    try {
        std::vector<float4> opos(nverts);
        for (uint32_t i = 0; i < nverts; i++)
            opos[i] = make_float4(verts[i].position[0], verts[i].position[1], verts[i].position[2], 0.f);
        HIPC(c, c->d_opos.alloc(nverts));
        HIPC(c, c->d_verts.alloc((size_t)nverts * 8));
        HIPC(c, c->d_idx.alloc(nidx));
        HIPC(c, c->d_matidx.alloc(T));
        HIPC(c, c->d_mats.alloc(nmats));
        HIPC(c, hipMemcpy(c->d_opos, opos.data(), sizeof(float4) * nverts, hipMemcpyHostToDevice));
        HIPC(c, hipMemcpy(c->d_verts, verts, sizeof(rtbvh_vertex) * nverts, hipMemcpyHostToDevice));
        HIPC(c, hipMemcpy(c->d_idx, indices, sizeof(uint32_t) * nidx, hipMemcpyHostToDevice));
        HIPC(c, hipMemcpy(c->d_matidx, mat_idx, sizeof(uint32_t) * T, hipMemcpyHostToDevice));
        HIPC(c, hipMemcpy(c->d_mats, mats, sizeof(rtbvh_material) * nmats, hipMemcpyHostToDevice));
        std::vector<uint4> info(ntex ? ntex : 1);
        size_t total = 0;
        for (uint32_t k = 0; k < ntex; k++) {
            info[k] = make_uint4((uint32_t)total, textures[k].width, textures[k].height, 0u);
            total += (size_t)textures[k].width * textures[k].height;
        }
        if (total >= (1ull << 32)) return fail(c, RTBVH_ERR_INVALID_ARG, "set_scene: textures too large");
        HIPC(c, c->d_texels.alloc(total ? total : 1));
        HIPC(c, c->d_texinfo.alloc(info.size()));
        for (uint32_t k = 0; k < ntex; k++)
            HIPC(c, hipMemcpy(c->d_texels + info[k].x, textures[k].rgba8,
                              (size_t)textures[k].width * textures[k].height * 4, hipMemcpyHostToDevice));
        HIPC(c, hipMemcpy(c->d_texinfo, info.data(), sizeof(uint4) * info.size(), hipMemcpyHostToDevice));
        if (!c->d_srgb) {
            float tab[256];
            rtbvh_srgb_table(tab);
            HIPC(c, c->d_srgb.alloc(256));
            HIPC(c, hipMemcpy(c->d_srgb, tab, sizeof(tab), hipMemcpyHostToDevice));
        }
        c->ntex = ntex;
    } catch (const std::bad_alloc&) {
        return fail(c, RTBVH_ERR_OOM, "set_scene: host allocation failed");
    }
    static_assert(sizeof(rtbvh_material) == sizeof(Mat), "material layout");
    c->V = nverts;
    c->T = T;
    c->nmat = nmats;
    TRY(ensure_build_capacity(c, T));
    if (c->cfg.morton_mode == RTBVH_MORTON_CPUTESTS) {
        BuildArgs a = build_args(c);
        launch_bounds(a, c->stream);
        TRY(check_launch(c, "mesh bounds"));
        HIPC(c, hipStreamSynchronize(c->stream));
    }
// ... 458 lines not shown
    if (!c->last.traced) return fail(c, RTBVH_ERR_NOT_READY, "no trace yet");
    if (!c->last.frame_here)
        return fail(c, RTBVH_ERR_NOT_READY, "the last trace was a band trace: the frame is elsewhere");
    HIPC(c, hipStreamSynchronize(c->stream));
    HIPC(c, hipMemcpy(rgba, c->d_color, sizeof(float4) * (size_t)c->last.W * c->last.H, hipMemcpyDeviceToHost));
    return RTBVH_OK;
}

rtbvh_status rtbvh_read_intensity(rtbvh_ctx* c, float* inten) {
    if (!c || !inten) return RTBVH_ERR_INVALID_ARG;
    if (!c->last.traced || !c->last.intensity_here) return fail(c, RTBVH_ERR_NOT_READY, "no full-frame trace yet");
    HIPC(c, hipStreamSynchronize(c->stream));
    HIPC(c, hipMemcpy(inten, c->d_intensity, sizeof(float) * (size_t)c->last.W * c->last.H, hipMemcpyDeviceToHost));
    return RTBVH_OK;
}

const float* rtbvh_framebuffer_device(rtbvh_ctx* c) { return c ? (const float*)c->d_color.h : nullptr; }

rtbvh_status rtbvh_read_bvh(rtbvh_ctx* c, rtbvh_node* out, uint32_t capacity) {
    if (!c || !out) return RTBVH_ERR_INVALID_ARG;
    if (!c->tree.built) return fail(c, RTBVH_ERR_NOT_READY, "no build yet");
    const size_t total = 2 * (size_t)c->T - 1;
    if (capacity < total) return fail(c, RTBVH_ERR_INVALID_ARG, "read_bvh: capacity < 2n-1");
    HIPC(c, hipSetDevice(c->cfg.device));
    void* tmp = nullptr;
    HIPC(c, hipMalloc(&tmp, total * sizeof(rtbvh_node)));
    BuildArgs a = build_args(c);
    launch_export(a, tmp, c->stream);
    hipError_t e1 = hipGetLastError();
    hipError_t e2 = hipStreamSynchronize(c->stream);
    hipError_t e3 = hipMemcpy(out, tmp, total * sizeof(rtbvh_node), hipMemcpyDeviceToHost);
    (void)hipFree(tmp);
    HIPC(c, e1);
    HIPC(c, e2);
    HIPC(c, e3);
    return RTBVH_OK;
}

rtbvh_status rtbvh_present(rtbvh_ctx* c, uint8_t* rgba8) {
    if (!c || !rgba8) return RTBVH_ERR_INVALID_ARG;
    if (!c->last.traced || !c->last.frame_here)
        return fail(c, RTBVH_ERR_NOT_READY, "present: no full frame on this context");
    HIPC(c, hipSetDevice(c->cfg.device));
    const size_t n = (size_t)c->last.W * c->last.H;
    uint32_t* d = nullptr;
    HIPC(c, hipMallocAsync((void**)&d, n * 4, c->stream));
    launch_present(c->d_color, c->last.W, c->last.H, d, c->stream);
    hipError_t e1 = hipGetLastError();
    hipError_t e2 = hipMemcpyAsync(rgba8, d, n * 4, hipMemcpyDeviceToHost, c->stream);
    hipError_t e3 = hipFreeAsync(d, c->stream);
    hipError_t e4 = hipStreamSynchronize(c->stream);
    HIPC(c, e1);
    HIPC(c, e2);
    HIPC(c, e3);
    HIPC(c, e4);
    return RTBVH_OK;
}

rtbvh_status rtbvh_read_wide(rtbvh_ctx* c, uint32_t* out, uint64_t capacity) {
    if (!c || !out) return RTBVH_ERR_INVALID_ARG;
    if (!c->tree.built) return fail(c, RTBVH_ERR_NOT_READY, "no build yet");
    const size_t total = c->T > 1 ? 2 * (size_t)(c->T - 1) : 0;
    if (capacity < total) return fail(c, RTBVH_ERR_INVALID_ARG, "read_wide: capacity < 2(n-1)");
    HIPC(c, hipSetDevice(c->cfg.device));
    TRY(ensure_form(c, RECORDS, c->stream));
    TRY(ensure_form(c, PSEUDO, c->stream));
    HIPC(c, hipStreamSynchronize(c->stream));
    if (total) HIPC(c, hipMemcpy(out, c->d_rec, total * sizeof(Inner), hipMemcpyDeviceToHost));
    return RTBVH_OK;
}

rtbvh_status rtbvh_read_qnodes(rtbvh_ctx* c, uint32_t* out, uint64_t capacity) {
    if (!c || !out) return RTBVH_ERR_INVALID_ARG;
    if (!c->tree.built) return fail(c, RTBVH_ERR_NOT_READY, "no build yet");
    const size_t total = c->T > 1 ? 2 * (size_t)c->T - 1 : 0;
    if (capacity < total) return fail(c, RTBVH_ERR_INVALID_ARG, "read_qnodes: capacity < 2n-1");
    HIPC(c, hipSetDevice(c->cfg.device));
    TRY(ensure_form(c, QNODES, c->stream));
    HIPC(c, hipStreamSynchronize(c->stream));
    if (total) HIPC(c, hipMemcpy(out, c->d_qnode, total * sizeof(QNode), hipMemcpyDeviceToHost));
    return RTBVH_OK;
}

rtbvh_status rtbvh_read_morton(rtbvh_ctx* c, uint32_t* codes) {
    if (!c || !codes) return RTBVH_ERR_INVALID_ARG;
    if (!c->tree.built) return fail(c, RTBVH_ERR_NOT_READY, "no build yet");
    HIPC(c, hipStreamSynchronize(c->stream));
    HIPC(c, hipMemcpy(codes, c->d_codes, sizeof(uint32_t) * c->T, hipMemcpyDeviceToHost));
    return RTBVH_OK;
}

rtbvh_status rtbvh_read_sorted(rtbvh_ctx* c, uint32_t* keys, uint32_t* ids) {
    if (!c) return RTBVH_ERR_INVALID_ARG;
    if (!c->tree.built) return fail(c, RTBVH_ERR_NOT_READY, "no build yet");
    HIPC(c, hipStreamSynchronize(c->stream));
    if (keys) HIPC(c, hipMemcpy(keys, c->sorted.keys, sizeof(uint32_t) * c->T, hipMemcpyDeviceToHost));
    if (ids) HIPC(c, hipMemcpy(ids, c->sorted.vals, sizeof(uint32_t) * c->T, hipMemcpyDeviceToHost));
    return RTBVH_OK;
}

rtbvh_status rtbvh_read_rays(rtbvh_ctx* c, rtbvh_ray_present* reflect_out, rtbvh_ray_present* refract_out) {
    if (!c) return RTBVH_ERR_INVALID_ARG;
    if (!c->last.traced || c->last.rec_P == 0)
        return fail(c, RTBVH_ERR_NOT_READY, "read_rays: the last trace ran without RTBVH_FLAG_REFRACT_RECORDS");
    HIPC(c, hipSetDevice(c->cfg.device));
    HIPC(c, hipStreamSynchronize(c->stream));
    const size_t bytes = c->last.rec_P * sizeof(rtbvh_ray_present);
    if (reflect_out) HIPC(c, hipMemcpy(reflect_out, c->d_refl_rec, bytes, hipMemcpyDeviceToHost));
    if (refract_out) HIPC(c, hipMemcpy(refract_out, c->d_refr_rec, bytes, hipMemcpyDeviceToHost));
    return RTBVH_OK;
}

rtbvh_status rtbvh_get_stats(rtbvh_ctx* c, rtbvh_stats* out) {
    if (!c || !out) return RTBVH_ERR_INVALID_ARG;
    memset(out, 0, sizeof(*out));
    if (rtbvh_status st = sync_all(c)) return st;
    out->num_tris = c->T;
    out->num_nodes = c->T ? 2 * c->T - 1 : 0;
    const LastTrace& t = c->last;
    const TraceSet& set = c->sets[t.slot];
    out->width = t.W;
    out->height = t.H;
    const uint32_t nb = c->n_builds < (uint32_t)rtbvh_ctx::RING ? c->n_builds : rtbvh_ctx::RING;
    for (uint32_t k = 0; k < nb; k++) {
        float ms;
        HIPC(c, hipEventElapsedTime(&ms, c->evb[k][0], c->evb[k][5]));
        out->ms_build += ms / nb;
        for (int st = 0; st < 5; st++) {
            HIPC(c, hipEventElapsedTime(&ms, c->evb[k][st], c->evb[k][st + 1]));
            out->ms_stage[st] += ms / nb;
        }
    }
    out->timed_builds = nb;
    const uint32_t nt = c->n_traces < (uint32_t)rtbvh_ctx::RING ? c->n_traces : rtbvh_ctx::RING;
    for (uint32_t k = 0; k < nt; k++) {
        float ms;
        HIPC(c, hipEventElapsedTime(&ms, c->evt[k][0], c->evt[k][2]));
        out->ms_trace += ms / nt;
        HIPC(c, hipEventElapsedTime(&ms, c->evt[k][0], c->evt[k][1]));
        out->ms_stage[5] += ms / nt;
        HIPC(c, hipEventElapsedTime(&ms, c->evt[k][1], c->evt[k][2]));
        out->ms_stage[6] += ms / nt;
        if (c->evt_trav[k]) {
            HIPC(c, hipEventElapsedTime(&ms, c->evt[k][3], c->evt[k][4]));
            out->ms_stage[7] += ms / nt;
        }
    }
    out->timed_traces = nt;
    if (t.traced && set.counters) {
        unsigned long long cnt[64];
        uint32_t q[32 * rtbvh_ctx::MAXSPLIT];
        HIPC(c, hipMemcpy(cnt, set.counters, sizeof(cnt), hipMemcpyDeviceToHost));
        HIPC(c, hipMemcpy(q, set.qcount, sizeof(uint32_t) * 32 * t.nsplit, hipMemcpyDeviceToHost));
        out->primary_rays = (uint64_t)t.W * deal_rows(t.H, t.rank, t.nranks, c->root_share);
        uint64_t b = 0;
        for (uint32_t g = 0; g < t.nsplit; g++)
            for (uint32_t k = 0; k < t.bounces; k++) b += q[32 * g + k];
        out->bounce_rays = b;
        for (int p = 0; p < 2; p++) {
            out->internal_visits[p] = cnt[2 + 3 * p];
            out->leaf_visits[p] = cnt[3 + 3 * p];
            out->hits[p] = cnt[4 + 3 * p];
        }
        out->stack_overflows = cnt[8];
        out->textured_hits = cnt[9];
        out->trav_wave_steps = cnt[10];
        out->trav_max_steps = cnt[13];
        out->trav_longest = cnt[20];
        for (int k = 0; k < 32; k++) out->trav_steps_log2[k] = cnt[32 + k];
        out->trav_mixed_steps = cnt[11];
        out->trav_active_lanes = cnt[12];
        for (int p = 0; p < 2; p++) {
            out->packet_steps[p] = cnt[14 + p];
            out->bin_entries[p] = cnt[16 + p];
        }
    }
    out->graph_captures = c->graph_captures;
    out->walk_flags = t.walk;
    out->walk_state = t.walk_state;
    out->cert_traces = c->cert_traces;
    if (t.traced && t.cert && set.qcount) {
        uint32_t q[32];
        HIPC(c, hipMemcpy(q, set.qcount, sizeof(q), hipMemcpyDeviceToHost));
        out->redo_rays[0] = q[16];
        for (uint32_t k = 0; k < t.bounces && k < 15; k++) out->redo_rays[1] += q[17 + k];
        for (uint32_t k = 0; k < t.bounces && k < 15; k++) {
            uint32_t nd = 0;
            HIPC(c, hipMemcpy(&nd, set.next + (size_t)NEXT_SEGS * NEXT_STRIDE * k + DEFER_COUNT, sizeof(nd),
                              hipMemcpyDeviceToHost));
            out->redo_rays[1] += nd;
            out->redo_deferred += nd;
        }
    }
    out->redo_total = out->redo_rays[0] + out->redo_rays[1];
    return RTBVH_OK;
}

uint64_t rtbvh_bin_builds(rtbvh_ctx* c) { return c ? c->bin_builds : 0; }

uint32_t rtbvh_bin_sets(rtbvh_ctx* c) {
    uint32_t n = 0;
    for (uint32_t k = 0; c && k < rtbvh_ctx::MAXSPLIT; k++) n += c->sets[k].pb.bins ? 1u : 0u;
    return n;
}

rtbvh_status rtbvh_set_flags(rtbvh_ctx* c, uint32_t flags) {
    if (!c) return RTBVH_ERR_INVALID_ARG;
    c->cfg.flags = flags;
    return RTBVH_OK;
}

rtbvh_status rtbvh_reset_stats(rtbvh_ctx* c) {
    if (!c) return RTBVH_ERR_INVALID_ARG;
    HIPC(c, hipStreamSynchronize(c->stream));
    c->n_builds = 0;
    c->n_traces = 0;
    return RTBVH_OK;
}

rtbvh_status rtbvh_sort_pairs_async(rtbvh_ctx* c, uint32_t* kin, uint32_t* vin, uint32_t* kout, uint32_t* vout,
                                    uint32_t n, uint32_t key_bits) {
    if (!c || (n && (!kin || !vin || !kout || !vout)) || key_bits == 0 || key_bits > 32)
        return RTBVH_ERR_INVALID_ARG;
    if (n == 0) return RTBVH_OK;
    HIPC(c, hipSetDevice(c->cfg.device));
    const uint32_t passes = (key_bits + RADIX_BITS - 1) / RADIX_BITS;
    uint32_t *tk = nullptr, *tv = nullptr, *scratch = nullptr;
    HIPC(c, hipMallocAsync((void**)&scratch, sort_scratch_words(n) * 4, c->stream));
    if (passes > 1) {
        HIPC(c, hipMallocAsync((void**)&tk, (size_t)n * 4, c->stream));
        HIPC(c, hipMallocAsync((void**)&tv, (size_t)n * 4, c->stream));
    }
    if (passes & 1) radix_sort_pairs(kin, vin, kout, vout, tk, tv, n, key_bits, scratch, c->stream);
    else radix_sort_pairs(kin, vin, tk, tv, kout, vout, n, key_bits, scratch, c->stream);
    rtbvh_status st = check_launch(c, "sort kernels");
    (void)hipFreeAsync(scratch, c->stream);
    if (tk) (void)hipFreeAsync(tk, c->stream);
    if (tv) (void)hipFreeAsync(tv, c->stream);
    return st;
}

rtbvh_status rtbvh_sort_pairs_host(rtbvh_ctx* c, const uint32_t* keys, const uint32_t* vals, uint32_t* kout,
                                   uint32_t* vout, uint32_t n, uint32_t key_bits) {
    if (!c || (n && (!keys || !vals || !kout || !vout))) return RTBVH_ERR_INVALID_ARG;
    if (n == 0) return RTBVH_OK;
    HIPC(c, hipSetDevice(c->cfg.device));
    uint32_t* d = nullptr;
    HIPC(c, hipMalloc((void**)&d, (size_t)n * 16));
    uint32_t *dk = d, *dv = d + n, *ok = d + 2 * (size_t)n, *ov = d + 3 * (size_t)n;
    rtbvh_status st = RTBVH_OK;
    if (hipMemcpy(dk, keys, (size_t)n * 4, hipMemcpyHostToDevice) != hipSuccess ||
        hipMemcpy(dv, vals, (size_t)n * 4, hipMemcpyHostToDevice) != hipSuccess)
        st = fail(c, RTBVH_ERR_HIP, "sort_pairs_host: upload failed");
    if (!st) st = rtbvh_sort_pairs_async(c, dk, dv, ok, ov, n, key_bits);
    if (!st && hipStreamSynchronize(c->stream) != hipSuccess) st = fail(c, RTBVH_ERR_HIP, "sort_pairs_host: sync");
    if (!st && (hipMemcpy(kout, ok, (size_t)n * 4, hipMemcpyDeviceToHost) != hipSuccess ||
                hipMemcpy(vout, ov, (size_t)n * 4, hipMemcpyDeviceToHost) != hipSuccess))
        st = fail(c, RTBVH_ERR_HIP, "sort_pairs_host: download failed");
    (void)hipFree(d);
    return st;
}

rtbvh_status rtbvh_build_from_codes(rtbvh_ctx* c, const uint32_t* sorted_codes, const float* leaf_boxes, uint32_t n,
                                    rtbvh_node* out) {
    if (!c || !sorted_codes || !leaf_boxes || !out || n == 0 || n >= (1u << 30)) return RTBVH_ERR_INVALID_ARG;
    HIPC(c, hipSetDevice(c->cfg.device));
    if (c->ev_query) HIPC(c, hipEventSynchronize(c->ev_query));
    c->query_busy = false;
    TRY(ensure_build_capacity(c, n));
    DevBuf<float> d_boxes;
    DevBuf<rtbvh_node> d_out;
    HIPC(c, d_boxes.alloc((size_t)n * 6));
    HIPC(c, d_out.alloc(2 * (size_t)n - 1));
    reset_tree(c);
    HIPC(c, hipMemcpy(c->d_ka, sorted_codes, (size_t)n * 4, hipMemcpyHostToDevice));
    HIPC(c, hipMemcpy(d_boxes, leaf_boxes, (size_t)n * 24, hipMemcpyHostToDevice));
    BuildArgs a = build_args(c);
// ... 1247 lines not shown
```

raytracebvh_amd/csrc/build.hip:

```cpp
#include "rtbvh_internal.h"

namespace rtbvh {
namespace {

#ifndef RTBVH_NT_STORES
#define RTBVH_NT_STORES 7
#endif
template <int BIT>
__device__ __forceinline__ void st_out(float4* p, float4 v) {
    typedef float v4 __attribute__((ext_vector_type(4)));
    if (RTBVH_NT_STORES & BIT) __builtin_nontemporal_store(v4{v.x, v.y, v.z, v.w}, reinterpret_cast<v4*>(p));
    else *p = v;
}

constexpr uint32_t BLOCK = 256;
#ifndef RTBVH_REFIT_BLOCK
#define RTBVH_REFIT_BLOCK 512
#endif
constexpr uint32_t RBLOCK = RTBVH_REFIT_BLOCK;
#ifndef RTBVH_REFIT_PROBE
#define RTBVH_REFIT_PROBE 0
#endif
#ifndef RTBVH_QSKIP
#define RTBVH_QSKIP 1
// ... 595 lines not shown
#pragma unroll
        for (int k = 0; k < 3; k++) {
            if ((uint32_t)k < n && !(E[k].id & LEAF_BIT)) {
                const float ar = half_area(E[k].b);
                if (ar > best) { best = ar; pick = k; }
            }
        }
        if (pick < 0) break;
        QEnt sel = E[0];
#pragma unroll
        for (int k = 1; k < 3; k++) qent_sel(sel, E[k], k == pick);
        QEnt c0, c1;
        kids(sel, c0, c1);
#pragma unroll
        for (int k = 0; k < 3; k++) qent_sel(E[k], c0, k == pick);
        qent_sel(E[2], c1, n == 2);
        qent_sel(E[3], c1, n == 3);
        ++n;
    }
    QEnt P[4] = {E[0], E[1], E[2], E[3]};
    if (n == 2) { P[1] = E[0]; P[2] = E[1]; P[3] = E[0]; }
    if (n == 3) P[3] = E[0];
    const bool absent1 = n == 2, absent3 = n < 4;
    float lx[4], ly[4], lz[4], hx[4], hy[4], hz[4];
    uint32_t id[4];
#pragma unroll
    for (int k = 0; k < 4; k++) {
        lx[k] = P[k].b[0]; ly[k] = P[k].b[1]; lz[k] = P[k].b[2];
        hx[k] = P[k].b[3]; hy[k] = P[k].b[4]; hz[k] = P[k].b[5];
        id[k] = (P[k].id & LEAF_BIT) ? P[k].id : P[k].slot;
    }
    if (absent1) id[1] = INVALID;
    if (absent3) id[3] = INVALID;
#pragma unroll
    for (int k = 0; k < 4; k++) ent[k] = P[k].id;
    if (absent1) ent[1] = INVALID;
    if (absent3) ent[3] = INVALID;
    qnode_words(lx, ly, lz, hx, hy, hz, make_uint4(id[0], id[1], id[2], id[3]), edge, out);
}
__device__ __forceinline__ void record_kids(const Inner* __restrict__ rec, uint32_t slot, QEnt& c0, QEnt& c1) {
    const float4* r = reinterpret_cast<const float4*>(rec + slot);
    const float4 w0 = r[0], w1 = r[1], w2 = r[2], w3 = r[3];
    const uint32_t own = __float_as_uint(w3.z);
    c0.id = __float_as_uint(w3.x);
    c1.id = __float_as_uint(w3.y);
    c0.slot = 2 * own;
    c1.slot = 2 * own + 1;
    c0.b[0] = w0.x; c0.b[1] = w0.y; c0.b[2] = w2.x; c0.b[3] = w0.z; c0.b[4] = w0.w; c0.b[5] = w2.y;
    c1.b[0] = w1.x; c1.b[1] = w1.y; c1.b[2] = w2.z; c1.b[3] = w1.z; c1.b[4] = w1.w; c1.b[5] = w2.w;
}
__device__ __forceinline__ void nbox_kids(const BuildArgs& a, uint32_t k, QEnt& c0, QEnt& c1) {
    const uint4 t = a.topo[k];
    c0.id = t.x;
    c1.id = t.y;
    c0.slot = 2 * k;
    c1.slot = 2 * k + 1;
    child_box(a, t.x, c0.b);
    child_box(a, t.y, c1.b);
}
template <bool PSEUDO_NOGRID = false>
__device__ __forceinline__ void qnode_from_records(Inner* __restrict__ rec, uint32_t slot, float E, QNode* dst) {
    QEnt e0, e1;
    record_kids(rec, slot, e0, e1);
    float4 w[4];
    uint32_t ent[4];
    greedy_qnode_words(e0, e1, [&](const QEnt& e, QEnt& c0, QEnt& c1) { record_kids(rec, e.slot, c0, c1); }, E, w,
                       ent);
    store4(dst, w);
    if (PSEUDO_NOGRID && w[0].w == 0.f) {
        f3 lo, hi;
        if (e0.id & LEAF_BIT) { ld_box(e0.b, lo, hi); store_pseudo_record(rec + e0.slot, e0.id, lo, hi); }
        if (e1.id & LEAF_BIT) { ld_box(e1.b, lo, hi); store_pseudo_record(rec + e1.slot, e1.id, lo, hi); }
    }
}

__global__ __launch_bounds__(BLOCK) void k_qnodes(Inner* __restrict__ rec, const uint32_t* __restrict__ pint,
                                                  const Inner* __restrict__ inner, QNode* __restrict__ qn, uint32_t T) {
    const uint32_t k = blockIdx.x * BLOCK + threadIdx.x;
    if (k + 1 >= T) return;
    const uint32_t slot = slot_of(pint[k], T);
    qnode_from_records(rec, slot, __uint_as_float(inner[k].aux0), qn + slot);
}

__device__ __forceinline__ void qnode_cross(const BuildArgs& a, uint32_t k) {
    const uint32_t slot = slot_of(a.pint[k], a.T);
    const float E = *node_edge(a, k);
    if (!a.rec_on) {
        QEnt e0, e1;
        nbox_kids(a, k, e0, e1);
        float4 w[4];
        uint32_t ent[4];
        greedy_qnode_words(e0, e1, [&](const QEnt& e, QEnt& c0, QEnt& c1) { nbox_kids(a, e.id, c0, c1); }, E, w, ent);
        store4(a.qnode + slot, w);
    } else if (a.pseudo) {
        qnode_from_records<false>(a.rec, slot, E, a.qnode + slot);
    } else {
        qnode_from_records<true>(a.rec, slot, E, a.qnode + slot);
    }
}
__global__ __launch_bounds__(BLOCK) void k_qnodes_late(BuildArgs a) {
    const uint32_t n = a.qlate[0];
    for (uint32_t j = blockIdx.x * BLOCK + threadIdx.x; j < n; j += gridDim.x * BLOCK) qnode_cross(a, a.qlate[1 + j]);
}

__global__ __launch_bounds__(BLOCK) void k_records(BuildArgs a) {
    const uint32_t k = blockIdx.x * BLOCK + threadIdx.x;
    if (k + 1 >= a.T) return;
    const uint4 t = a.topo[k];
    float l[6], r[6];
    child_box(a, t.x, l);
    child_box(a, t.y, r);
    f3 l0, l1, r0, r1;
    ld_box(l, l0, l1);
    ld_box(r, r0, r1);
    const uint32_t slot = slot_of(a.pint[k], a.T);
    store_record(a.rec + slot, l0, l1, r0, r1, t.x, t.y, k);
    if (a.qnode && reinterpret_cast<const float4*>(a.qnode + slot)[0].w == 0.f) {
        if (t.x & LEAF_BIT) store_leaf_record(a.rec, k, 0, t.x, l0, l1);
        if (t.y & LEAF_BIT) store_leaf_record(a.rec, k, 1, t.y, r0, r1);
    }
}
__global__ __launch_bounds__(BLOCK) void k_nbox(BuildArgs a) {
    const uint32_t k = blockIdx.x * BLOCK + threadIdx.x;
    if (k + 1 >= a.T) return;
    const Inner* r = a.rec + slot_of(a.pint[k], a.T);
    float l[6], q[6];
    record_box(r, 0, l);
    record_box(r, 1, q);
    f3 l0, l1, r0, r1;
    ld_box(l, l0, l1);
    ld_box(q, r0, r1);
    st_nbox(a.nbox, k, vmin(l0, r0), vmax(l1, r1));
}

template <bool PSEUDO>
__global__ __launch_bounds__(RBLOCK) void k_refit(BuildArgs a) {
    __shared__ uint32_t s_cnt[RBLOCK];
    __shared__ __align__(16) float s_box[RBLOCK * 12 >= RTBVH_REFIT_STAGE_SLOTS * 16 ? RBLOCK
                                                                                  : RTBVH_REFIT_STAGE_SLOTS * 16 / 12 + 1][2][6];
    static_assert(sizeof(float) * 12 * RBLOCK >= 16 * 128 * (RBLOCK / 64), "leaf staging fits in s_box");
    __shared__ uint4 s_topo[RBLOCK];
    __shared__ uint32_t s_pint[RBLOCK];
    __shared__ uint32_t s_xn;
    __shared__ uint32_t s_own[RTBVH_REFIT_STAGE_SLOTS / 32];
    __shared__ float s_topo_z[3 * (RBLOCK / 64)];
    const uint32_t T = a.T;
    const uint32_t base = blockIdx.x * RBLOCK, tid = threadIdx.x;
    const uint32_t i = base + tid;
    const uint32_t end = base + RBLOCK;
    s_cnt[tid] = 0;
    if (tid == 0) s_xn = 0;
    if (i == 0 && a.qlate) a.qlate[0] = 0;
    if (i + 1 < T) {
        s_topo[tid] = a.topo[i];
        s_pint[tid] = a.pint[i];
    }
    f3 lo = mk(0.f, 0.f, 0.f), hi = lo;
    uint32_t e = INVALID;
    float emax = 0.f;
    {
        float4 r[4] = {};
        if (i < T) {
            leaf_record_words(a, i, lo, hi, r);
            float zkey;
#if RTBVH_REFIT_PROBE == 5
            zkey = lo.z;
#else
            leaf_margin(r, lo.z, hi.z, emax, zkey);
            a.lfp[i] = leaf_footprint(lo, hi, zkey);
#endif
        }
        const uint32_t w0 = base + (tid & ~63u);
        if (RTBVH_REFIT_PROBE != 4) staged_records(a.leaf + 4 * (size_t)w0, T > w0 ? min(64u, T - w0) : 0u, r,
                       reinterpret_cast<float4*>(&s_box[0][0][0]) + 128 * (tid >> 6));
    }
    if (i < T) {
// ... 523 lines not shown
        if (e == INVALID) {
            st_rootbox(a, lo, hi);
            a.rootbox[6] = lo.z; a.rootbox[7] = hi.z;
        }
    }
    __syncthreads();
    for (uint32_t p = tid; p + 1 < T; p += SMALL_BLOCK) {
        f3 l0, l1, r0, r1;
        ld_box(s_box[p][0], l0, l1);
        ld_box(s_box[p][1], r0, r1);
        const uint2 ids = s_ids[p];
        store_record(a.rec + slot_of(s_pint[p], T), l0, l1, r0, r1, ids.x, ids.y, p);
        *node_edge(a, p) = __uint_as_float(s_cnt[p] & 0x7FFFFFFFu);
    }
#ifdef RTBVH_SMALL_PROBE
    SMALL_MARK(6);
    if (tid == 0)
        printf("SMALLPROBE T=%u bounds %llu morton %llu sort %llu leaves+karras %llu links %llu refit %llu (x10ns)\n", T,
               (unsigned long long)(tmark[1] - tmark[0]), (unsigned long long)(tmark[2] - tmark[1]),
               (unsigned long long)(tmark[3] - tmark[2]), (unsigned long long)(tmark[4] - tmark[3]),
               (unsigned long long)(tmark[5] - tmark[4]), (unsigned long long)(tmark[6] - tmark[5]));
#endif
}

template <uint32_t KPT>
__global__ __launch_bounds__(SMALL_BLOCK) void k_morton_sort_small(BuildArgs a, uint32_t* __restrict__ sk,
                                                                   uint32_t* __restrict__ sv) {
    __shared__ uint64_t s_kv[KPT * SMALL_BLOCK];
    const uint32_t tid = threadIdx.x, T = a.T;
    uint64_t e[KPT];
#pragma unroll
    for (uint32_t b = 0; b < KPT; b++) {
        const uint32_t t = KPT * tid + b;
        e[b] = t < T ? ((uint64_t)morton_tri(a, t) << 32 | t) : ~0ull;
    }
    bitonic_sort(e, s_kv, tid);
#pragma unroll
    for (uint32_t b = 0; b < KPT; b++) {
        const uint32_t i = KPT * tid + b;
        if (i < T) {
            sk[i] = (uint32_t)(e[b] >> 32);
            sv[i] = (uint32_t)e[b];
        }
    }
}

struct RefNode { uint32_t parent, child_l, child_r, code; float bb_min[3], bb_max[3]; uint32_t index; };
static_assert(sizeof(RefNode) == 44, "44-B Node");

__global__ __launch_bounds__(BLOCK) void k_export(BuildArgs a, RefNode* __restrict__ out) {
    const uint32_t T = a.T;
    const uint32_t r = blockIdx.x * BLOCK + threadIdx.x;
    if (r >= 2 * T - 1) return;
    RefNode o;
    float box[6];
    uint32_t e;
    if (r < T) {
        e = T == 1 ? INVALID : a.pleaf[r];
        o.child_l = INVALID;
        o.child_r = INVALID;
        o.code = a.sorted_keys[r];
        o.index = a.leaf ? 3u * (__float_as_uint(a.leaf[4 * (size_t)r + 2].y) & ~LEAF_BIT) : 0u;
    } else {
        const uint32_t k = r - T;
        e = a.pint[k];
        const uint32_t cl = a.topo[k].x, cr = a.topo[k].y;
        o.child_l = (cl & LEAF_BIT) ? (cl & ~LEAF_BIT) : T + cl;
        o.child_r = (cr & LEAF_BIT) ? (cr & ~LEAF_BIT) : T + cr;
        o.code = 0;
        o.index = 0;
    }
    if (e == INVALID) {
        o.parent = INVALID;
        for (int k = 0; k < 6; k++) box[k] = a.rootbox[k];
    } else {
        o.parent = (e >> 1) + T;
        if (a.rec_on) record_box(a.rec + slot_of(a.pint[e >> 1], T), e & 1u, box);
        else child_box(a, r < T ? LEAF_BIT | r : r - T, box);
    }
    for (int k = 0; k < 3; k++) { o.bb_min[k] = box[k]; o.bb_max[k] = box[3 + k]; }
    out[r] = o;
}

inline uint32_t blocks_for(size_t n) { return (uint32_t)((n + BLOCK - 1) / BLOCK); }

}

void launch_bounds(const BuildArgs& a, hipStream_t s) {
    uint32_t blocks = blocks_for(a.V);
    if (blocks > BOUNDS_BLOCKS) blocks = BOUNDS_BLOCKS;
    if (blocks == 0) blocks = 1;
    hipLaunchKernelGGL(k_bounds, dim3(blocks), dim3(BLOCK), 0, s, a.opos, a.V, a.bounds);
    hipLaunchKernelGGL(k_bounds_final, dim3(1), dim3(BLOCK), 0, s, a.bounds, blocks);
}
void launch_update_vertices(const VertexUpdate& u, hipStream_t s) {
    uint32_t blocks = blocks_for(u.count);
    if (blocks > BOUNDS_BLOCKS) blocks = BOUNDS_BLOCKS;
    if (u.bounds && u.first == 0 && u.count == u.V) {
        hipLaunchKernelGGL(k_update_vertices<true>, dim3(blocks), dim3(BLOCK), 0, s, u);
        hipLaunchKernelGGL(k_bounds_final, dim3(1), dim3(BLOCK), 0, s, u.bounds, blocks);
        return;
    }
    hipLaunchKernelGGL(k_update_vertices<false>, dim3(blocks), dim3(BLOCK), 0, s, u);
    if (u.bounds) {
        BuildArgs a{};
        a.opos = u.opos;
        a.V = u.V;
        a.bounds = u.bounds;
        launch_bounds(a, s);
    }
}
void launch_morton(const BuildArgs& a, hipStream_t s) {
    hipLaunchKernelGGL(k_morton<true>, dim3(blocks_for(a.T)), dim3(BLOCK), 0, s, a);
}
void launch_clip(const BuildArgs& a, hipStream_t s) {
    hipLaunchKernelGGL(k_morton<false>, dim3(blocks_for(a.T)), dim3(BLOCK), 0, s, a);
}
void launch_karras(const BuildArgs& a, hipStream_t s) {
    if (a.T < 2) return;
    if (a.delta_mode == 0) hipLaunchKernelGGL(k_karras<0>, dim3(blocks_for(a.T)), dim3(BLOCK), 0, s, a);
    else hipLaunchKernelGGL(k_karras<1>, dim3(blocks_for(a.T)), dim3(BLOCK), 0, s, a);
}
uint32_t small_build_max() { return SMALL_T; }
uint32_t small_sort_max() { return 8 * SMALL_BLOCK; }
static void launch_one_workgroup(void (*kernel)(BuildArgs, uint32_t*, uint32_t*), const BuildArgs& a, hipStream_t s) {
    hipLaunchKernelGGL(kernel, dim3(1), dim3(SMALL_BLOCK), 0, s, a, const_cast<uint32_t*>(a.sorted_keys),
                       const_cast<uint32_t*>(a.sorted_vals));
}
void launch_morton_sort_small(const BuildArgs& a, hipStream_t s) {
    launch_one_workgroup(a.T <= 4 * SMALL_BLOCK ? k_morton_sort_small<4> : k_morton_sort_small<8>, a, s);
}
void launch_build_small(const BuildArgs& a, hipStream_t s) {
    launch_one_workgroup(a.delta_mode == 0 ? k_build_small<0> : k_build_small<1>, a, s);
}
void launch_qnodes(const BuildArgs& a, hipStream_t s) {
    if (a.T > 1)
        hipLaunchKernelGGL(k_qnodes, dim3((a.T - 1 + BLOCK - 1) / BLOCK), dim3(BLOCK), 0, s, a.rec, a.pint, a.inner,
                           a.qnode, a.T);
}
uint32_t refit_blocks(uint32_t T) { return (T + RBLOCK - 1) / RBLOCK; }
__global__ __launch_bounds__(1024) void k_zrange(const float* __restrict__ zpart, uint32_t nb, float* __restrict__ rootbox) {
    __shared__ float s_z[3 * 16];
    float zl = INFINITY, zh = -INFINITY, em = 0.f;
    for (uint32_t b = threadIdx.x; b < nb; b += 1024) {
        zl = fminf(zl, zpart[ZPART * b]);
        zh = fmaxf(zh, zpart[ZPART * b + 1]);
        em = fmaxf(em, zpart[ZPART * b + 2]);
    }
    reduce_zrange_block<16>(zl, zh, em, s_z);
    if (threadIdx.x == 0) {
        rootbox[6] = zl;
        rootbox[7] = zh;
        rootbox[8] = em;
    }
}
void launch_refit_leaves(const BuildArgs& a, hipStream_t s) {
    const uint32_t nb = refit_blocks(a.T);
    if (a.pseudo) hipLaunchKernelGGL(k_refit<true>, dim3(nb), dim3(RBLOCK), 0, s, a);
    else hipLaunchKernelGGL(k_refit<false>, dim3(nb), dim3(RBLOCK), 0, s, a);
    hipLaunchKernelGGL(k_zrange, dim3(1), dim3(1024), 0, s, a.zpart, nb, a.rootbox);
}
static uint32_t launch_refit_group(const BuildArgs& a, hipStream_t s) {
    if (a.T <= RBLOCK) return 0;
    const uint32_t nb = refit_blocks(a.T);
    hipLaunchKernelGGL(k_refit_group, dim3((nb + RGROUP - 1) / RGROUP), dim3(GBLOCK), 0, s, a);
    return min(1024u, (nb + 15) / 16);
}
void launch_pb_count_top(const BuildArgs& b, const TraceArgs& a, uint32_t* off, uint32_t* cur, uint4* bins, uint32_t cap,
// ... 36 lines not shown
```

raytracebvh_amd/csrc/rtbvh_internal.h:

```cpp
#pragma once
#include <hip/hip_runtime.h>
#include <stdint.h>

#include "rtbvh_device.h"

namespace rtbvh {

#ifndef RTBVH_BOUNCE_WAVES
#define RTBVH_BOUNCE_WAVES 8
#endif
constexpr uint32_t BOUNCE_WAVES = RTBVH_BOUNCE_WAVES;

constexpr uint32_t SORT_BLOCK = 256;
#ifndef RTBVH_SORT_ITEMS
#define RTBVH_SORT_ITEMS 16
#endif
constexpr uint32_t SORT_ITEMS = RTBVH_SORT_ITEMS;
constexpr uint32_t SORT_TILE = SORT_BLOCK * SORT_ITEMS;
#ifndef RTBVH_RADIX_BITS
#define RTBVH_RADIX_BITS 8
#endif
constexpr uint32_t RADIX_BITS = RTBVH_RADIX_BITS;
constexpr uint32_t RADIX = 1u << RADIX_BITS;
constexpr size_t BOUNDS_WORDS = 8 + 6 * 1024;
constexpr uint32_t ROOTBOX_WORDS = 16;
constexpr uint32_t ZPART = 3;

inline uint32_t sort_tiles(uint32_t n) { return (n + SORT_TILE - 1) / SORT_TILE; }
inline size_t sort_scratch_words(uint32_t n) { return (size_t)RADIX * sort_tiles(n) + RADIX; }

struct SortResult { uint32_t* keys; uint32_t* vals; };
SortResult radix_sort_pairs(const uint32_t* kin, const uint32_t* vin, uint32_t* ka, uint32_t* va, uint32_t* kb,
                            uint32_t* vb, uint32_t n, uint32_t key_bits, uint32_t* scratch, hipStream_t s);

struct BuildArgs {
    const float4* opos;
    const uint32_t* idx;
    const uint32_t* matidx;
    uint32_t V, T;
    int morton_mode, delta_mode;
    const float* cam;
    float smin[3], smax[3];
    float* bounds;
    uint32_t* keys;
    uint32_t* vals;
    float4* tclip;
    const uint32_t* sorted_keys;
    const uint32_t* sorted_vals;
    float4* leaf;
    Inner* inner;
    uint4* topo;
    Inner* rec;
    uint32_t* pleaf;
    uint32_t* pint;
    uint32_t* refit_cnt;
    uint32_t* xlist;
    uint32_t* xcnt;
    float* rootbox;
    QNode* qnode;
    uint4* lfp;
    float* zpart;
    uint32_t pseudo;
    uint32_t rec_on;
    uint32_t* qlate;
    float* nbox;
};
void launch_bounds(const BuildArgs& a, hipStream_t s);
void launch_morton(const BuildArgs& a, hipStream_t s);
void launch_clip(const BuildArgs& a, hipStream_t s);
struct VertexUpdate {
    const float* pos;
    uint32_t pos_stride;
    const float* nrm;
    uint32_t nrm_stride;
    uint32_t first, count;
    float4* opos;
    float* verts;
    float* bounds;
    uint32_t V;
};
void launch_update_vertices(const VertexUpdate& u, hipStream_t s);
void launch_karras(const BuildArgs& a, hipStream_t s);
void launch_refit_leaves(const BuildArgs& a, hipStream_t s);
void launch_refit_tail(const BuildArgs& a, hipStream_t s);
void launch_pseudo(const BuildArgs& a, hipStream_t s);
uint32_t refit_blocks(uint32_t T);
void launch_qnodes(const BuildArgs& a, hipStream_t s);
uint32_t small_build_max();
void launch_build_small(const BuildArgs& a, hipStream_t s);
uint32_t small_sort_max();
void launch_morton_sort_small(const BuildArgs& a, hipStream_t s);
void launch_records(const BuildArgs& a, hipStream_t s);
void launch_nbox(const BuildArgs& a, hipStream_t s);
void launch_export(const BuildArgs& a, void* out_nodes, hipStream_t s);
void launch_from_codes(const BuildArgs& a, const float* leaf_boxes, hipStream_t s);

struct TraceArgs {
    const Inner* inner;
    const uint4* topo;
    const float* nbox;
    bool nb;
    const float4* leaf;
    const float4* tclip;
    const float* verts;
    const uint32_t* idx;
    const uint32_t* matidx;
    const Mat* mats;
    const uint32_t* texels;
    const uint4* texinfo;
    const float* srgb;
    uint32_t ntex;
    uint32_t T, W, H, rank, nranks;
    uint32_t band0, bstep;
    uint32_t my_bands;
    const uint32_t* band_list;
    const uint32_t* band_slots;
    const uint32_t* pb_gate;
    uint32_t pb_cap, pb_ntx;
    const float* rootbox;
    const uint4* lfp;
    const float* cam;
    float4* color;
    float* intensity;
    unsigned long long* counters;
    unsigned long long* overflow;
    int stack_limit, stack_limit4;
    int stack_limit4b;
    bool limited;
    bool acyclic;
    float* refl_rec;
    float* refr_rec;
    const QNode* qnode;
    uint32_t* pb_list;
};
enum class PrimaryKind { LANE_REFERENCE, LANE_NEAREST, PACKET_REFERENCE, PACKET_NEAREST, PACKET_WIDE, BINNED };
enum class BounceWalk { REFERENCE, NEAREST, WIDE_QUANTIZED };
void launch_primary(const TraceArgs& a, RayQ* q, uint32_t* qcount, bool count, bool emit, PrimaryKind kind,
                    hipStream_t s);
struct Redo {
    uint32_t* list;
    uint32_t* count;
    uint32_t* defer = nullptr;
    const uint32_t* dnext = nullptr;
};
constexpr uint32_t REDO_BLOCKS = 512;
constexpr uint32_t PB_TILE = 32;
constexpr uint32_t PB_NZ = 16;
constexpr uint32_t PB_LEAVES = 1024;
constexpr uint32_t PB_LISTS = 16, PB_LIST_STRIDE = 32;
inline __host__ __device__ uint32_t pb_list_cap(uint32_t T) {
    return ((T + PB_LEAVES - 1) / PB_LEAVES + PB_LISTS - 1) / PB_LISTS * PB_LEAVES;
}
inline size_t pb_list_words(uint32_t T) { return (size_t)PB_LISTS * PB_LIST_STRIDE + (size_t)PB_LISTS * pb_list_cap(T); }
struct PrimBins {
    uint32_t* off;
    uint32_t* cur;
    uint4* bins;
    unsigned long long* keys;
    uint32_t* sums;
    uint32_t cap, ntx, nty;
};
inline uint32_t pb_tiles_x(uint32_t W) { return (W + PB_TILE - 1) / PB_TILE; }
inline uint32_t pb_tiles_y(uint32_t rows) { return (rows + PB_TILE - 1) / PB_TILE; }
void launch_pb_bins(const TraceArgs& a, const PrimBins& pb, uint32_t rows, bool zeroed, hipStream_t s,
                    const BuildArgs* tail = nullptr);
void launch_pb_raster(const TraceArgs& a, const PrimBins& pb, uint32_t rows, RayQ* q, uint32_t* qcount, bool count,
                      bool emit, hipStream_t s, const Redo* redo = nullptr, bool small_tiles = false);
bool pb_keys_used();
void launch_pb_count_top(const BuildArgs& b, const TraceArgs& a, uint32_t* off, uint32_t* cur, uint4* bins, uint32_t cap,
                         uint32_t ntx, uint32_t leaf_blocks, hipStream_t s);
void launch_pb_gate(const TraceArgs& a, const PrimBins& pb, RayQ* q, uint32_t* qcount, bool count, bool emit,
                    hipStream_t s, bool reference);
struct ZeroList {
    static constexpr int N = 5;
    uint32_t* ptr[N];
    size_t words[N];
};
void launch_zero(const ZeroList& z, hipStream_t s);
void launch_bounce(const TraceArgs& a, const RayQ* qin, const uint32_t* qin_count, const uint32_t* perm, RayQ* qout,
                   uint32_t* qout_count, bool count, bool emit, bool nearest, hipStream_t s);
#ifndef RTBVH_NEXT_SEGS
#define RTBVH_NEXT_SEGS 64
#endif
constexpr uint32_t NEXT_SEGS = RTBVH_NEXT_SEGS;
constexpr uint32_t NEXT_STRIDE = 32;
constexpr uint32_t NEXT_WORDS = 16 * NEXT_SEGS * NEXT_STRIDE;
constexpr uint32_t DEFER_CLAIM = 1, DEFER_COUNT = 2;
constexpr uint32_t DEFER_VALID = 0x80000000u;
struct BounceShade {
    RayQ* qout;
    uint32_t* qout_count;
    bool emit;
    uint32_t* redo;
    uint32_t* redo_count;
    uint32_t P;
};
void launch_bounce_traverse(const TraceArgs& a, const RayQ* qin, const uint32_t* qin_count, const uint32_t* perm,
                            bool count, BounceWalk walk, float2* hitrec, uint32_t* next, uint32_t blocks,
                            hipStream_t s, bool cert = false, uint32_t* defer = nullptr, const BounceShade* es = nullptr);
void launch_bounce_shade(const TraceArgs& a, const RayQ* qin, const uint32_t* qin_count, const float2* hitrec,
                         RayQ* qout, uint32_t* qout_count, bool count, bool emit, uint32_t P, hipStream_t s,
                         const Redo* redo = nullptr);
struct CameraWords { float w[32]; };
void launch_set_camera(const float* wvp, const float* wv, float* cam, hipStream_t s);
void launch_count_diff(const float4* a, const float4* b, size_t n, unsigned long long* diff, hipStream_t s);
void launch_assemble(const float4* bands, const uint32_t* slots, uint32_t stride_rows, uint32_t W, uint32_t H,
                     uint32_t nranks,
                     float4* frame, hipStream_t s);
void launch_present(const float4* color, uint32_t W, uint32_t H, uint32_t* out, hipStream_t s);
void launch_bounce_keys(const RayQ* q, const uint32_t* count, const float* box, uint32_t P, uint32_t* keys,
                        uint32_t* vals, hipStream_t s);

struct QueryArgs {
    const Inner* inner;
    const uint4* topo;
// ... 276 lines not shown
```

raytracebvh_amd/csrc/trace.hip:

```cpp
#include "rtbvh_internal.h"

#include <type_traits>

namespace rtbvh {
namespace {

constexpr uint32_t BLOCK = 256;
constexpr float EPSILON = 0.01f;

struct Counts { uint32_t internal, leaf, overflow, wint, wleaf; };

typedef float f2v __attribute__((ext_vector_type(2)));
typedef float v4f __attribute__((ext_vector_type(4)));

__device__ __forceinline__ uint32_t child_slot(uint32_t id, uint32_t own, uint32_t side) {
    return (id & LEAF_BIT) ? id : 2 * own + side;
}
__device__ __forceinline__ uint32_t root_slot(uint32_t T) { return T == 1 ? LEAF_BIT : 2 * T - 2; }

__device__ __forceinline__ void pin(float4& a) {
    float x = a.x, y = a.y, z = a.z, w = a.w;
    asm volatile("" : "+v"(x), "+v"(y), "+v"(z), "+v"(w));
    a = make_float4(x, y, z, w);
}
// ... 3917 lines not shown

void launch_pb_bins(const TraceArgs& a, const PrimBins& pb, uint32_t rows, bool zeroed, hipStream_t s,
                    const BuildArgs* tail) {
    if (rows == 0 || a.W == 0 || a.T == 0) return;
    const uint32_t keys = pb.ntx * pb.nty * PB_NZ;
    if (!zeroed) (void)hipMemsetAsync(pb.off, 0, ((size_t)keys + 1) * sizeof(uint32_t), s);
    if (!zeroed && a.pb_list) (void)hipMemsetAsync(a.pb_list, 0, (size_t)PB_LISTS * PB_LIST_STRIDE * sizeof(uint32_t), s);
    const dim3 lg((a.T + PB_LEAVES - 1) / PB_LEAVES);
    if (tail) launch_pb_count_top(*tail, a, pb.off, pb.cur, pb.bins, pb.cap, pb.ntx, lg.x, s);
    else hipLaunchKernelGGL((k_pb_bin<false>), lg, dim3(BLOCK), 0, s, a, pb.off, pb.cur, pb.bins, pb.cap, pb.ntx);
    const uint32_t sb = (keys + PB_SCAN - 1) / PB_SCAN;
    hipLaunchKernelGGL(k_pb_sums, dim3(sb), dim3(PB_SCAN), 0, s, pb.off, pb.sums, keys);
    hipLaunchKernelGGL(k_pb_scan, dim3(sb), dim3(PB_SCAN), 0, s, pb.off, pb.cur, pb.sums, keys);
    hipLaunchKernelGGL((k_pb_bin<true>), lg, dim3(BLOCK), 0, s, a, pb.off, pb.cur, pb.bins, pb.cap, pb.ntx);
}

void launch_pb_raster(const TraceArgs& a, const PrimBins& pb, uint32_t rows, RayQ* q, uint32_t* qcount, bool count,
                      bool emit, hipStream_t s, const Redo* redo, bool small_tiles) {
    if (rows == 0 || a.W == 0 || a.T == 0) return;
    const dim3 grid(pb.ntx, pb.nty);
    uint32_t* rl = redo ? redo->list : nullptr;
    uint32_t* rc = redo ? redo->count : nullptr;
    const bool rec = a.refl_rec || a.refr_rec;
    const auto raster = [&](auto* kernel, uint32_t rb) {
        hipLaunchKernelGGL(kernel, grid, dim3(rb), 0, s, a, pb.off, pb.bins, pb.cap, pb.ntx, rows, pb.keys, q, qcount,
                           (int)emit, rl, rc);
    };
#if RTBVH_PB_FUSE
    with_bools([&](auto COUNT, auto CERT) {
        if (rec) raster(k_primary_binned<COUNT, CERT, true, true>, PB_RASTER_BLOCK);
        else if (small_tiles)
            raster(k_primary_binned<COUNT, CERT, true, false, PB_RASTER_BLOCK_SMALL>, PB_RASTER_BLOCK_SMALL);
        else raster(k_primary_binned<COUNT, CERT, true, false>, PB_RASTER_BLOCK);
    }, count, redo != nullptr);
#else
    (void)rec;
    (void)small_tiles;
    with_bools([&](auto COUNT) { raster(k_primary_binned<COUNT, false, false, true>, PB_RASTER_BLOCK); }, count);
    with_bools([&](auto COUNT, auto CERT) {
        hipLaunchKernelGGL((k_pb_shade<COUNT, CERT>), grid, dim3(PB_SHADE_BLOCK), 0, s, a, pb.off, pb.cap, pb.ntx, rows,
                           pb.keys, q, qcount, (int)emit, rl, rc);
    }, count, redo != nullptr);
#endif
    if (redo) {
        with_bools([&](auto COUNT) {
            hipLaunchKernelGGL((k_primary_redo<COUNT>), dim3(REDO_BLOCKS), dim3(BLOCK), 0, s, a, rl, rc, q, qcount, (int)emit);
        }, count);
    }
}

void launch_pb_gate(const TraceArgs& a, const PrimBins& pb, RayQ* q, uint32_t* qcount, bool count, bool emit,
                    hipStream_t s, bool reference) {
    if (a.W == 0 || a.T == 0) return;
    TraceArgs g = a;
    g.pb_gate = pb.off;
    g.pb_cap = pb.cap;
    g.pb_ntx = pb.ntx;
    launch_primary(g, q, qcount, count, emit, reference ? PrimaryKind::LANE_REFERENCE : PrimaryKind::LANE_NEAREST, s);
}

void launch_bounce(const TraceArgs& a, const RayQ* qin, const uint32_t* qin_count, const uint32_t* perm, RayQ* qout,
                   uint32_t* qout_count, bool count, bool emit, bool nearest, hipStream_t s) {
    const uint32_t blocks = 2048;
    with_bools([&](auto COUNT, auto NEAREST, auto LIM) {
        hipLaunchKernelGGL((k_bounce<COUNT, NEAREST, LIM>), dim3(blocks), dim3(BLOCK), 0, s, a, qin, qin_count, perm, qout,
                           qout_count, (int)emit);
    }, count, nearest, a.limited);
}

void launch_bounce_keys(const RayQ* q, const uint32_t* count, const float* box, uint32_t P, uint32_t* keys,
                        uint32_t* vals, hipStream_t s) {
    hipLaunchKernelGGL(k_bounce_keys, dim3((P + BLOCK - 1) / BLOCK), dim3(BLOCK), 0, s, q, count, box, P, keys, vals);
}

void launch_bounce_traverse(const TraceArgs& a, const RayQ* qin, const uint32_t* qin_count, const uint32_t* perm,
                            bool count, BounceWalk walk, float2* hitrec, uint32_t* next, uint32_t blocks,
                            hipStream_t s, bool cert, uint32_t* defer, const BounceShade* es) {
    if (blocks == 0) blocks = 2048;
    const bool wide = walk == BounceWalk::WIDE_QUANTIZED;
    const bool certified = wide && cert;
    const bool early = RTBVH_EARLY_SHADE && certified && es;
    const uint32_t nshade = early ? (es->P + ESHADE_RAYS - 1) / ESHADE_RAYS : 0u;
    if (early) hipLaunchKernelGGL(k_hit_init, dim3(1024), dim3(BLOCK), 0, s, hitrec, qin_count);
    const auto launch = [&](auto* kernel) {
        hipLaunchKernelGGL(kernel, dim3(blocks + nshade), dim3(BLOCK), 0, s, a.inner, a.qnode, a.leaf, a.T, qin, qin_count,
                           perm, hitrec, next, a.counters, a.overflow, wide ? a.stack_limit4b : a.stack_limit, defer,
                           a.topo, a.nb ? a.nbox : nullptr, blocks, a, early ? es->qout : nullptr,
                           early ? es->qout_count : nullptr, early ? (int)es->emit : 0, early ? es->redo : nullptr,
                           early ? es->redo_count : nullptr);
    };
    const bool guard = count || !a.acyclic;
    if (certified)
        with_bools([&](auto COUNT, auto GUARD, auto ES) { launch(k_bounce_trav<COUNT, 2, false, GUARD, true, ES>); }, count,
                   guard, early);
    else if (wide)
        with_bools([&](auto COUNT, auto LIM, auto GUARD) { launch(k_bounce_trav<COUNT, 2, LIM, GUARD>); }, count, a.limited,
                   guard);
    else
        with_bools([&](auto COUNT, auto NEAREST, auto LIM, auto GUARD) {
            launch(k_bounce_trav<COUNT, NEAREST ? 1 : 0, LIM, GUARD>);
        }, count, walk == BounceWalk::NEAREST, a.limited, guard);
}

void launch_bounce_shade(const TraceArgs& a, const RayQ* qin, const uint32_t* qin_count, const float2* hitrec,
                         RayQ* qout, uint32_t* qout_count, bool count, bool emit, uint32_t P, hipStream_t s,
                         const Redo* redo) {
    if (P == 0) return;
    uint32_t* rl = redo ? redo->list : nullptr;
    uint32_t* rc = redo ? redo->count : nullptr;
    const dim3 g((P + BLOCK - 1) / BLOCK);
    with_bools([&](auto COUNT, auto CERT) {
        hipLaunchKernelGGL((k_bounce_shade<COUNT, CERT>), g, dim3(BLOCK), 0, s, a, qin, qin_count, hitrec, qout, qout_count,
                           (int)emit, rl, rc);
    }, count, redo != nullptr);
    if (redo)
        with_bools([&](auto COUNT) {
            hipLaunchKernelGGL((k_bounce_redo<COUNT>), dim3(REDO_BLOCKS), dim3(BLOCK), 0, s, a, qin, rl, rc, qout,
                               qout_count, (int)emit, redo->defer, redo->dnext);
        }, count);
}

void launch_assemble(const float4* bands, const uint32_t* slots, uint32_t stride_rows, uint32_t W, uint32_t H,
                     uint32_t nranks, float4* frame, hipStream_t s) {
    const size_t n = (size_t)W * H;
    hipLaunchKernelGGL(k_assemble, dim3((uint32_t)((n + BLOCK - 1) / BLOCK)), dim3(BLOCK), 0, s, bands, slots,
                       stride_rows, W, H, nranks, frame);
}

void launch_present(const float4* color, uint32_t W, uint32_t H, uint32_t* out, hipStream_t s) {
    const size_t n = (size_t)W * H;
    if (n) hipLaunchKernelGGL(k_present, dim3((uint32_t)((n + BLOCK - 1) / BLOCK)), dim3(BLOCK), 0, s, color, W, H, out);
}

__global__ __launch_bounds__(64) void k_set_camera(CameraWords m, float* __restrict__ cam) {
    if (threadIdx.x < 32) cam[threadIdx.x] = m.w[threadIdx.x];
}

void launch_set_camera(const float* wvp, const float* wv, float* cam, hipStream_t s) {
    CameraWords m;
    for (int i = 0; i < 16; i++) {
        m.w[i] = wvp[i];
        m.w[16 + i] = wv[i];
    }
    hipLaunchKernelGGL(k_set_camera, dim3(1), dim3(64), 0, s, m, cam);
}

void launch_count_diff(const float4* a, const float4* b, size_t n, unsigned long long* diff, hipStream_t s) {
    if (n == 0) return;
    size_t blocks = (n + BLOCK - 1) / BLOCK;
    if (blocks > 4096) blocks = 4096;
    hipLaunchKernelGGL(k_count_diff, dim3((uint32_t)blocks), dim3(BLOCK), 0, s, reinterpret_cast<const uint4*>(a),
                       reinterpret_cast<const uint4*>(b), n, diff);
}

}
```

raytracebvh_amd/graphics.py:

```python
from __future__ import annotations

import ctypes
import os

import numpy as np

from . import _lib as _L
from .scene import EYE_REFERENCE, Scene, camera_look, camera_orbit, camera_reference


def _is_tensor(x) -> bool:
    return type(x).__module__.split(".")[0] == "torch" and hasattr(x, "data_ptr")


def make_rays(origins, directions, t_max=float("inf")):
    if _is_tensor(origins) or _is_tensor(directions):
        import torch
        dev = origins.device if _is_tensor(origins) else directions.device
        o = torch.as_tensor(origins, dtype=torch.float32, device=dev).reshape(-1, 3)
        d = torch.as_tensor(directions, dtype=torch.float32, device=dev).reshape(-1, 3)
        if o.shape != d.shape:
            raise ValueError(f"make_rays: {tuple(o.shape)} origins and {tuple(d.shape)} directions")
        rays = torch.zeros((o.shape[0], 8), dtype=torch.float32, device=dev)
        rays[:, 0:3] = o
# ... 944 lines not shown
        if hasattr(stream, "cuda_stream"):
            return stream
        return torch.cuda.ExternalStream(int(stream), device=device) if int(stream) else torch.cuda.default_stream(device)

    def _signed_on_stream(self, pts, mode, stream, read):
        import torch
        ts = self._torch_stream(stream, pts.device)
        with torch.cuda.stream(ts):
            rec = torch.empty((len(pts), 8), dtype=torch.float32, device=pts.device)
            self.signed(pts, None, mode, out=rec, stream=ts)
            return read(rec)

    def signed_distance(self, points, max_dist2=None, mode: int = 0, stream=None):
        mode = mode & ~_L.SIGNED_INSIDE_ONLY
        if _is_tensor(points):
            import torch
            _, pts = check_nearest_points(points, float("inf") if max_dist2 is None else max_dist2,
                                          getattr(self, "device", None))

            def read(rec):
                d2 = rec[:, 3]
                d = torch.where(d2 < 0, torch.full_like(d2, float("nan")), torch.sqrt(d2.clamp(min=0)))
                inside = (rec[:, 7].contiguous().view(torch.int32) & 1) != 0
                return torch.where(inside, -d, d)
            return self._signed_on_stream(pts, mode, stream, read)
        rec = self.signed(points, max_dist2, mode)
        with np.errstate(invalid="ignore"):
            d = np.where(rec["tri"] == 0xFFFFFFFF, np.float32(np.nan), np.sqrt(rec["dist2"]))
        return np.where(rec["flags"] & 1, -d, d).astype(np.float32)

    def inside(self, points, vote3: bool = False, mode: int = 0, stream=None):
        mode = mode | _L.SIGNED_INSIDE_ONLY | (_L.SIGNED_VOTE3 if vote3 else 0)
        if _is_tensor(points):
            import torch
            _, pts = check_nearest_points(points, float("inf"), getattr(self, "device", None))
            return self._signed_on_stream(pts, mode, stream,
                                          lambda rec: (rec[:, 7].contiguous().view(torch.int32) & 1) != 0)
        return (self.signed(points, None, mode)["flags"] & 1).astype(bool)

    def signed_counts(self) -> dict:
        out = np.zeros(4, np.uint64)
        self._check(_L.lib().rtbvh_signed_counts(self._h, _L.ptr(out)))
        return dict(zip(("points", "inside", "internal_steps", "leaf_steps"), (int(v) for v in out)))

    def read_framebuffer(self) -> np.ndarray:
        out = np.zeros((self.height, self.width, 4), np.float32)
        self._check(_L.lib().rtbvh_read_framebuffer(self._h, _L.ptr(out)))
        return out

    def read_rays(self):
        refl = np.zeros((self.height, self.width, 14), np.float32)
        refr = np.zeros((self.height, self.width, 14), np.float32)
        self._check(_L.lib().rtbvh_read_rays(self._h, _L.ptr(refl), _L.ptr(refr)))
        return refl, refr

    def present(self) -> np.ndarray:
        out = np.zeros((self.height, self.width, 4), np.uint8)
        self._check(_L.lib().rtbvh_present(self._h, _L.ptr(out)))
        return out

    def read_intensity(self) -> np.ndarray:
        out = np.zeros((self.height, self.width), np.float32)
        self._check(_L.lib().rtbvh_read_intensity(self._h, _L.ptr(out)))
        return out

    def framebuffer_device_ptr(self) -> int:
        return _L.lib().rtbvh_framebuffer_device(self._h) or 0

    def read_bvh(self) -> np.ndarray:
        out = np.zeros(2 * self.num_tris - 1, dtype=_L.NODE_DTYPE)
        self._check(_L.lib().rtbvh_read_bvh(self._h, ctypes.c_void_p(out.ctypes.data), len(out)))
        return out

    def read_wide(self) -> np.ndarray:
        out = np.zeros((max(2 * (self.num_tris - 1), 0), 16), np.uint32)
        self._check(_L.lib().rtbvh_read_wide(self._h, _L.ptr(out), len(out)))
        return out

    def read_qnodes(self) -> np.ndarray:
        out = np.zeros((max(2 * self.num_tris - 1, 0) if self.num_tris > 1 else 0, 16), np.uint32)
        self._check(_L.lib().rtbvh_read_qnodes(self._h, _L.ptr(out), len(out)))
        return out

    def read_morton(self) -> np.ndarray:
        out = np.zeros(self.num_tris, np.uint32)
        self._check(_L.lib().rtbvh_read_morton(self._h, _L.ptr(out)))
        return out

    def read_sorted(self):
        keys = np.zeros(self.num_tris, np.uint32)
        ids = np.zeros(self.num_tris, np.uint32)
        self._check(_L.lib().rtbvh_read_sorted(self._h, _L.ptr(keys), _L.ptr(ids)))
        return keys, ids

    def stats(self) -> dict:
        s = _L.Stats()
        self._check(_L.lib().rtbvh_get_stats(self._h, ctypes.byref(s)))
        return s.as_dict()

    def reset_stats(self):
        self._check(_L.lib().rtbvh_reset_stats(self._h))

    def set_flags(self, flags: int):
        self._check(_L.lib().rtbvh_set_flags(self._h, flags))

    def bin_builds(self) -> int:
        return int(_L.lib().rtbvh_bin_builds(self._h))

    def bin_sets(self) -> int:
        return int(_L.lib().rtbvh_bin_sets(self._h))

    def sort_pairs(self, keys: np.ndarray, vals: np.ndarray, key_bits: int = 32):
        keys = np.ascontiguousarray(keys, np.uint32)
        vals = np.ascontiguousarray(vals, np.uint32)
        ko = np.zeros_like(keys)
        vo = np.zeros_like(vals)
        self._check(_L.lib().rtbvh_sort_pairs_host(self._h, _L.ptr(keys), _L.ptr(vals), _L.ptr(ko), _L.ptr(vo),
                                                   len(keys), key_bits))
        return ko, vo

    def sort_pairs_device(self, keys_ptr: int, vals_ptr: int, keys_out_ptr: int, vals_out_ptr: int, n: int,
                          key_bits: int = 32):
        self._check(_L.lib().rtbvh_sort_pairs_async(self._h, ctypes.c_void_p(keys_ptr), ctypes.c_void_p(vals_ptr),
                                                    ctypes.c_void_p(keys_out_ptr), ctypes.c_void_p(vals_out_ptr),
                                                    n, key_bits))

    def build_from_codes(self, sorted_codes: np.ndarray, leaf_boxes: np.ndarray) -> np.ndarray:
        codes = np.ascontiguousarray(sorted_codes, np.uint32)
        boxes = np.ascontiguousarray(leaf_boxes, np.float32).reshape(-1, 6)
        out = np.zeros(2 * len(codes) - 1, dtype=_L.NODE_DTYPE)
        self._check(_L.lib().rtbvh_build_from_codes(self._h, _L.ptr(codes), _L.ptr(boxes), len(codes),
                                                    ctypes.c_void_p(out.ctypes.data)))
        return out


class Graphics:

    def __init__(self, width: int = 800, height: int = 800, bounces: int = 3, **ctx_kwargs):
        self.width, self.height, self.bounces = width, height, bounces
        self.eye = np.array(EYE_REFERENCE, np.float32)
        self.ctx = Context(**ctx_kwargs)

    def onInit(self, scene: Scene):
        self.ctx.set_scene(scene)

    def onUpdate(self):
        wvp, wv = camera_look(self.eye, self.width, self.height)
        self.ctx.set_camera(wvp, wv)
        self.computeBVH()

    def onKeyDown(self, key: int):
        self.eye = camera_orbit(self.eye, key)

    def computeBVH(self):
        self.ctx.compute_bvh(self.width, self.height, self.bounces)

    def framebuffer(self) -> np.ndarray:
        return self.ctx.read_framebuffer()

    def onRender(self) -> np.ndarray:
        return self.ctx.present()

    def save_bmp(self, path: str):
        save_bmp(path, self.onRender())

    def onDestroy(self):
# ... 17 lines not shown
```

Baseline: 5224 Mrays/s.

## Build a binned-SAH walk-only quantized tree for certified bounce traversal

Adds a secondary walk-only BVH. Subtrees of at most 512 leaves under the LBVH are rebuilt per workgroup in shared memory with a 16-bin SAH split under a depth budget, then quantized into a separate QNode array that the certified wide bounce traversal uses. It is built lazily, on the third trace of the same build epoch or when forced by env, and cached until the next build. The aim is fewer node visits on bounce rays in exchange for extra build kernels, memory, and an unfused tail on the pass that builds it.

```diff
diff --git a/include/rtbvh.h b/include/rtbvh.h
--- a/include/rtbvh.h
+++ b/include/rtbvh.h
@@ -113,6 +113,9 @@
     uint64_t redo_rays[2];
     uint64_t trav_longest;
     uint64_t redo_deferred;
+    uint64_t walk_tree_builds;
+    uint32_t walk_tree_used;
+    uint32_t reserved_walk_tree;
 } rtbvh_stats;
 typedef struct rtbvh_ctx rtbvh_ctx;
 
@@ -354,6 +357,7 @@
 rtbvh_status rtbvh_read_bvh(rtbvh_ctx* ctx, rtbvh_node* out, uint32_t capacity);
 rtbvh_status rtbvh_read_wide(rtbvh_ctx* ctx, uint32_t* records, uint64_t capacity);
 rtbvh_status rtbvh_read_qnodes(rtbvh_ctx* ctx, uint32_t* nodes, uint64_t capacity);
+rtbvh_status rtbvh_read_walk_qnodes(rtbvh_ctx* ctx, uint32_t* nodes, uint64_t capacity);
 rtbvh_status rtbvh_read_morton(rtbvh_ctx* ctx, uint32_t* codes);
 rtbvh_status rtbvh_read_sorted(rtbvh_ctx* ctx, uint32_t* sorted_codes, uint32_t* tri_ids);
 rtbvh_status rtbvh_read_rays(rtbvh_ctx* ctx, rtbvh_ray_present* reflect_out, rtbvh_ray_present* refract_out);
diff --git a/raytracebvh_amd/_lib.py b/raytracebvh_amd/_lib.py
--- a/raytracebvh_amd/_lib.py
+++ b/raytracebvh_amd/_lib.py
@@ -28,7 +28,7 @@
     "rtbvh_trace_async", "rtbvh_compute_bvh", "rtbvh_trace_band_async", "rtbvh_band_rows", "rtbvh_verify_walk",
     "rtbvh_deal_bands", "rtbvh_deal_rows", "rtbvh_set_band_deal",
     "rtbvh_synchronize", "rtbvh_read_framebuffer", "rtbvh_read_intensity", "rtbvh_framebuffer_device",
-    "rtbvh_read_bvh", "rtbvh_read_wide", "rtbvh_read_qnodes", "rtbvh_read_morton", "rtbvh_read_sorted", "rtbvh_read_rays", "rtbvh_get_stats",
+    "rtbvh_read_bvh", "rtbvh_read_wide", "rtbvh_read_qnodes", "rtbvh_read_walk_qnodes", "rtbvh_read_morton", "rtbvh_read_sorted", "rtbvh_read_rays", "rtbvh_get_stats",
     "rtbvh_reset_stats", "rtbvh_set_flags", "rtbvh_bin_builds", "rtbvh_bin_sets",
     "rtbvh_sort_pairs_async", "rtbvh_sort_pairs_host", "rtbvh_build_from_codes", "rtbvh_scene_load_obj",
     "rtbvh_scene_synthetic", "rtbvh_scene_free", "rtbvh_scene_num_vertices", "rtbvh_scene_num_indices",
@@ -137,7 +137,9 @@
                 ("walk_state", ctypes.c_uint32), ("packet_steps", ctypes.c_uint64 * 2),
                 ("cert_traces", ctypes.c_uint64), ("redo_total", ctypes.c_uint64),
                 ("bin_entries", ctypes.c_uint64 * 2), ("redo_rays", ctypes.c_uint64 * 2),
-                ("trav_longest", ctypes.c_uint64), ("redo_deferred", ctypes.c_uint64)]
+                ("trav_longest", ctypes.c_uint64), ("redo_deferred", ctypes.c_uint64),
+                ("walk_tree_builds", ctypes.c_uint64), ("walk_tree_used", ctypes.c_uint32),
+                ("reserved_walk_tree", ctypes.c_uint32)]
 
     def as_dict(self) -> dict:
         d = {}
@@ -202,6 +204,7 @@
         "rtbvh_read_morton": (i32, [vp, vp]),
         "rtbvh_read_wide": (i32, [vp, vp, ctypes.c_uint64]),
         "rtbvh_read_qnodes": (i32, [vp, vp, ctypes.c_uint64]),
+        "rtbvh_read_walk_qnodes": (i32, [vp, vp, ctypes.c_uint64]),
         "rtbvh_read_sorted": (i32, [vp, vp, vp]),
         "rtbvh_read_rays": (i32, [vp, vp, vp]),
         "rtbvh_get_stats": (i32, [vp, ctypes.POINTER(Stats)]),
diff --git a/raytracebvh_amd/csrc/api.hip b/raytracebvh_amd/csrc/api.hip
--- a/raytracebvh_amd/csrc/api.hip
+++ b/raytracebvh_amd/csrc/api.hip
@@ -106,6 +106,23 @@
     bool valid = false;
     Event filled;
     uint32_t readers = 0;
+};
+
+struct WalkTreeBufs {
+    Grown<uint4> topo;
+    Grown<uint32_t> pint, roots;
+    Grown<float> nbox, edge;
+    Grown<QNode> qnode;
+    bool valid = false;
+    uint64_t epoch = 0;
+    uint32_t T = 0;
+    Event ready;
+    uint64_t seen_epoch = 0;
+    uint32_t passes = 0;
+    void reset() {
+        topo.reset(); pint.reset(); roots.reset(); nbox.reset(); edge.reset(); qnode.reset();
+        valid = false;
+    }
 };
 
 struct TraceSet {
@@ -136,6 +153,7 @@
     bool cert = false;
     bool frame_here = false;
     bool intensity_here = false;
+    bool walk_tree = false;
 };
 
 struct rtbvh_ctx {
@@ -200,6 +218,9 @@
     uint64_t bins_epoch = 1;
     uint64_t bin_builds = 0;
     bool knob_bins_reuse = true;
+    WalkTreeBufs wt;
+    int knob_walk_tree = -1;
+    uint64_t walk_tree_builds = 0;
     LastTrace last;
 
     static constexpr int RING = 32;
@@ -352,6 +373,7 @@
     if (T <= c->cap_T && c->d_codes) return RTBVH_OK;
     drop_graph(c);
     reset_tree(c);
+    c->wt.reset();
     const size_t n = T, ni = T > 1 ? T - 1 : 1;
     HIPC(c, c->d_codes.alloc(n));
     HIPC(c, c->d_ids.alloc(n));
@@ -766,7 +788,43 @@
     bool inflight, fuse_tail, overlap, small_tiles, early_shade;
     uint32_t bset;
     bool fill_bins;
+    bool walk_tree;
 };
+
+int plan_walk_tree(rtbvh_ctx* c, const WalkPlan& p) {
+    if (c->capturing || c->knob_walk_tree == 0 || c->T < 2) return 0;
+    if (!(p.cert && p.bounces > 0 && p.wk.refill && p.wk.bounce == BounceWalk::WIDE_QUANTIZED)) return 0;
+    WalkTreeBufs& w = c->wt;
+    if (w.seen_epoch != c->bins_epoch) {
+        w.seen_epoch = c->bins_epoch;
+        w.passes = 0;
+    }
+    w.passes++;
+    if (w.valid && w.epoch == c->bins_epoch && w.T == c->T) return 1;
+    return c->knob_walk_tree == 1 || w.passes >= 3 ? 2 : 0;
+}
+rtbvh_status make_walk_tree(rtbvh_ctx* c) {
+    WalkTreeBufs& w = c->wt;
+    const size_t T = c->T, ni = T - 1;
+    w.valid = false;
+    HIPC(c, w.topo.reserve(ni));
+    HIPC(c, w.pint.reserve(ni));
+    HIPC(c, w.nbox.reserve(6 * ni));
+    HIPC(c, w.edge.reserve(ni));
+    HIPC(c, w.qnode.reserve(2 * T - 1));
+    HIPC(c, w.roots.reserve(2 + T / 2));
+    if (!w.ready) HIPC(c, hipEventCreateWithFlags(w.ready.out(), hipEventDisableTiming));
+    BuildArgs a = build_args(c);
+    a.nbox = c->d_nbox;
+    launch_walk_tree(a, WalkTree{w.topo, w.pint, w.nbox, w.edge, w.qnode, w.roots}, c->stream);
+    HIPC(c, hipGetLastError());
+    HIPC(c, hipEventRecord(w.ready, c->stream));
+    w.valid = true;
+    w.epoch = c->bins_epoch;
+    w.T = c->T;
+    c->walk_tree_builds++;
+    return RTBVH_OK;
+}
 
 WalkPlan plan_walks(const rtbvh_ctx* c, const TraceArgs& a, uint32_t bounces, hipStream_t s, uint32_t slot,
                     uint32_t flags, bool cert, bool timed, bool tail_pending, bool leaf_pending) {
@@ -817,6 +875,8 @@
         a.refl_rec = c->d_refl_rec;
         a.refr_rec = c->d_refr_rec;
     }
+    const int wt = plan_walk_tree(c, p);
+    if (wt == 2) p.fuse_tail = false;
     if (!p.fuse_tail && tail.pending) {
         tail.run();
         TRY(order_after_context(c, s));
@@ -825,6 +885,12 @@
     a.nb = p.cert;
     TRY(ensure_split_capacity(c, p.slot ? p.slot + 1 : p.nsplit, p.Pg));
     if (p.bounces > 0 && p.wk.refill && p.wk.bounce == BounceWalk::WIDE_QUANTIZED) TRY(ensure_form(c, QNODES, s));
+    if (wt) {
+        if (wt == 2) TRY(make_walk_tree(c));
+        if (s != c->stream) HIPC(c, hipStreamWaitEvent(s, c->wt.ready, 0));
+        a.qnode_walk = c->wt.qnode;
+        p.walk_tree = true;
+    }
     if (p.pkind == PrimaryKind::PACKET_REFERENCE || p.pkind == PrimaryKind::PACKET_NEAREST ||
         p.pkind == PrimaryKind::PACKET_WIDE)
         TRY(ensure_form(c, PSEUDO, s));
@@ -1008,7 +1074,7 @@
     TRY(launch_walks(c, p, a, tail));
     const bool frame_here = color == c->d_color && nranks == 1;
     c->last = LastTrace{true, W, H, bounces, rank, nranks, p.nsplit, slot, p.records ? p.P : 0, flags & WALK_FLAGS,
-                        walk_state, cert, frame_here, frame_here && inten != nullptr};
+                        walk_state, cert, frame_here, frame_here && inten != nullptr, p.walk_tree};
     return check_launch(c, "trace kernels");
 }
 
@@ -1146,6 +1212,7 @@
     if (const char* e = getenv("RTBVH_EARLY_SHADE")) c->knob_no_early_shade = atoi(e) == 0;
     if (const char* e = getenv("RTBVH_PB_SMALL_TILES")) c->knob_no_small_tiles = atoi(e) == 0;
     if (const char* e = getenv("RTBVH_BINS_REUSE")) c->knob_bins_reuse = atoi(e) != 0;
+    if (const char* e = getenv("RTBVH_WALK_TREE")) c->knob_walk_tree = atoi(e) != 0 ? 1 : 0;
     *out = c;
     return RTBVH_OK;
 }
@@ -1770,6 +1837,19 @@
     return RTBVH_OK;
 }
 
+rtbvh_status rtbvh_read_walk_qnodes(rtbvh_ctx* c, uint32_t* out, uint64_t capacity) {
+    if (!c || !out) return RTBVH_ERR_INVALID_ARG;
+    const WalkTreeBufs& w = c->wt;
+    if (!c->tree.built || !(w.valid && w.epoch == c->bins_epoch && w.T == c->T))
+        return fail(c, RTBVH_ERR_NOT_READY, "read_walk_qnodes: no walk-only tree of the current build");
+    const uint64_t total = 2 * (uint64_t)c->T - 1;
+    if (capacity < total) return fail(c, RTBVH_ERR_INVALID_ARG, "read_walk_qnodes: capacity < 2n-1");
+    HIPC(c, hipSetDevice(c->cfg.device));
+    HIPC(c, hipStreamSynchronize(c->stream));
+    HIPC(c, hipMemcpy(out, w.qnode, total * sizeof(QNode), hipMemcpyDeviceToHost));
+    return RTBVH_OK;
+}
+
 rtbvh_status rtbvh_read_morton(rtbvh_ctx* c, uint32_t* codes) {
     if (!c || !codes) return RTBVH_ERR_INVALID_ARG;
     if (!c->tree.built) return fail(c, RTBVH_ERR_NOT_READY, "no build yet");
@@ -1881,6 +1961,8 @@
         }
     }
     out->redo_total = out->redo_rays[0] + out->redo_rays[1];
+    out->walk_tree_builds = c->walk_tree_builds;
+    out->walk_tree_used = t.traced && t.walk_tree ? 1u : 0u;
     return RTBVH_OK;
 }
 
diff --git a/raytracebvh_amd/csrc/build.hip b/raytracebvh_amd/csrc/build.hip
--- a/raytracebvh_amd/csrc/build.hip
+++ b/raytracebvh_amd/csrc/build.hip
@@ -701,16 +701,19 @@
     qnode_from_records(rec, slot, __uint_as_float(inner[k].aux0), qn + slot);
 }
 
+__device__ __forceinline__ void qnode_nbox(const BuildArgs& a, uint32_t k, float E) {
+    QEnt e0, e1;
+    nbox_kids(a, k, e0, e1);
+    float4 w[4];
+    uint32_t ent[4];
+    greedy_qnode_words(e0, e1, [&](const QEnt& e, QEnt& c0, QEnt& c1) { nbox_kids(a, e.id, c0, c1); }, E, w, ent);
+    store4(a.qnode + slot_of(a.pint[k], a.T), w);
+}
 __device__ __forceinline__ void qnode_cross(const BuildArgs& a, uint32_t k) {
     const uint32_t slot = slot_of(a.pint[k], a.T);
     const float E = *node_edge(a, k);
     if (!a.rec_on) {
-        QEnt e0, e1;
-        nbox_kids(a, k, e0, e1);
-        float4 w[4];
-        uint32_t ent[4];
-        greedy_qnode_words(e0, e1, [&](const QEnt& e, QEnt& c0, QEnt& c1) { nbox_kids(a, e.id, c0, c1); }, E, w, ent);
-        store4(a.qnode + slot, w);
+        qnode_nbox(a, k, E);
     } else if (a.pseudo) {
         qnode_from_records<false>(a.rec, slot, E, a.qnode + slot);
     } else {
@@ -1400,8 +1403,275 @@
     out[r] = o;
 }
 
+constexpr uint32_t WT_K = 512;
+constexpr uint32_t WT_BLOCK = 256, WT_WAVES = WT_BLOCK / 64;
+constexpr int WT_NB = 16;
+constexpr int WT_DEPTH = 32;
+constexpr int WT_LEVELS = 64;
+static_assert(RBLOCK <= WT_K, "a node of more than WT_K leaves crosses a refit workgroup: its edge bound is in inner[]");
+static_assert(WT_K <= 65536 && WT_K % 2 == 0, "positions are 16-bit");
+
+__device__ __forceinline__ uint32_t wt_ord(float f) {
+    const uint32_t u = __float_as_uint(f);
+    return u ^ ((u >> 31) ? 0xFFFFFFFFu : 0x80000000u);
+}
+__device__ __forceinline__ float wt_unord(uint32_t u) {
+    return __uint_as_float(u ^ ((u >> 31) ? 0x80000000u : 0xFFFFFFFFu));
+}
+__device__ __forceinline__ int wt_clog2(uint32_t m) { return m <= 1 ? 0 : 32 - __clz(m - 1); }
+__device__ __forceinline__ void wt_wave_sync() {
+    __builtin_amdgcn_fence(__ATOMIC_RELEASE, "wavefront");
+    __builtin_amdgcn_wave_barrier();
+    __builtin_amdgcn_fence(__ATOMIC_ACQUIRE, "wavefront");
+}
+__device__ __forceinline__ float wt_first(float x) {
+    return __uint_as_float(__builtin_amdgcn_readfirstlane(__float_as_uint(x)));
+}
+__device__ __forceinline__ int wt_bin(float lo, float hi, float cl, float sc) {
+    return (int)fminf(fmaxf((0.5f * (lo + hi) - cl) * sc, 0.f), (float)(WT_NB - 1));
+}
+
+__global__ __launch_bounds__(BLOCK) void k_wt_select(BuildArgs a, WalkTree w) {
+    const uint32_t k = blockIdx.x * BLOCK + threadIdx.x;
+    if (k + 1 >= a.T) return;
+    const uint4 t = a.topo[k];
+    const uint32_t e = a.pint[k];
+    if (t.w - t.z + 1 > WT_K || t.z > t.w || t.w >= a.T) {
+        w.topo[k] = t;
+        w.pint[k] = e;
+        float b[6];
+        ld_nbox(a.nbox, k, b);
+        st_nbox(w.nbox, k, mk(b[0], b[1], b[2]), mk(b[3], b[4], b[5]));
+        w.edge[k] = *node_edge(a, k);
+        return;
+    }
+    bool root = e == INVALID;
+    if (!root) {
+        const uint4 p = a.topo[e >> 1];
+        root = p.w - p.z + 1 > WT_K;
+    }
+    if (root) {
+        w.pint[k] = e;
+        w.roots[1 + atomicAdd(&w.roots[0], 1u)] = k;
+    }
+}
+
+__global__ __launch_bounds__(WT_BLOCK) void k_wt_rebuild(BuildArgs a, WalkTree w) {
+    __shared__ float s_box[6][WT_K];
+    __shared__ float s_edge[WT_K];
+    __shared__ uint16_t s_perm[2][WT_K];
+    __shared__ uint32_t s_seg[2][WT_K / 2][2];
+    __shared__ uint32_t s_nseg[2];
+    __shared__ int s_budget;
+    __shared__ uint32_t s_bin[WT_WAVES][3][WT_NB][7];
+    const uint32_t tid = threadIdx.x, lane = tid & 63u, wave = tid >> 6;
+    const uint32_t nroots = min(w.roots[0], a.T / 2);
+    for (uint32_t r = blockIdx.x; r < nroots; r += gridDim.x) {
+        __syncthreads();
+        const uint32_t k0 = w.roots[1 + r];
+        const uint4 t0 = a.topo[k0];
+        const uint32_t lo = t0.z, n = min(t0.w - t0.z + 1, WT_K);
+        for (uint32_t i = tid; i < n; i += WT_BLOCK) {
+            const float4* rec = a.leaf + 4 * (size_t)(lo + i);
+            const float4 r0 = rec[0], r1 = rec[1], r2 = rec[2], r3 = rec[3];
+            s_box[0][i] = r2.z; s_box[1][i] = r2.w; s_box[2][i] = r3.x;
+            s_box[3][i] = r3.y; s_box[4][i] = r3.z; s_box[5][i] = r3.w;
+            s_edge[i] = mt_edge_bound(r0.w, r1.x, r1.y, r1.z, r1.w, r2.x);
+            s_perm[0][i] = (uint16_t)i;
+        }
+        if (tid == 0) {
+            int depth = 0;
+            for (uint32_t e = a.pint[k0]; e != INVALID && depth < WT_LEVELS; e = a.pint[e >> 1]) ++depth;
+            s_budget = max(min(WT_DEPTH + wt_clog2(WT_K), WT_LEVELS - depth), wt_clog2(n));
+            s_seg[0][0][0] = (n - 1) << 16;
+            s_seg[0][0][1] = k0;
+            s_nseg[0] = 1;
+            s_nseg[1] = 0;
+        }
+        __syncthreads();
+        for (int level = 0; level < WT_LEVELS; level++) {
+            const uint32_t cur = level & 1, nxt = cur ^ 1u;
+            const uint32_t ns = min(s_nseg[cur], WT_K / 2);
+            if (ns == 0) break;
+            for (uint32_t sg = wave; sg < ns; sg += WT_WAVES) {
+                const uint32_t ab = s_seg[cur][sg][0], id = s_seg[cur][sg][1];
+                const uint32_t pa = ab & 0xFFFFu, pb = ab >> 16, m = pb - pa + 1;
+                f3 bl = mk(INFINITY, INFINITY, INFINITY), bh = mk(-INFINITY, -INFINITY, -INFINITY), cl = bl, ch = bh;
+                float em = 0.f;
+                bool fin = true;
+                for (uint32_t p = pa + lane; p <= pb; p += 64) {
+                    const uint32_t j = s_perm[0][p];
+                    const f3 l = mk(s_box[0][j], s_box[1][j], s_box[2][j]), h = mk(s_box[3][j], s_box[4][j], s_box[5][j]);
+                    bl = vmin(bl, l);
+                    bh = vmax(bh, h);
+                    const f3 c = mk(0.5f * (l.x + h.x), 0.5f * (l.y + h.y), 0.5f * (l.z + h.z));
+                    cl = vmin(cl, c);
+                    ch = vmax(ch, c);
+                    em = fmaxf(em, s_edge[j]);
+                    fin = fin && fabsf(l.x) < INFINITY && fabsf(l.y) < INFINITY && fabsf(l.z) < INFINITY &&
+                          fabsf(h.x) < INFINITY && fabsf(h.y) < INFINITY && fabsf(h.z) < INFINITY;
+                }
+                for (int off = m >= 64 ? 32 : (1 << wt_clog2(m)) >> 1; off > 0; off >>= 1) {
+                    bl = vmin(bl, mk(__shfl_xor(bl.x, off, 64), __shfl_xor(bl.y, off, 64), __shfl_xor(bl.z, off, 64)));
+                    bh = vmax(bh, mk(__shfl_xor(bh.x, off, 64), __shfl_xor(bh.y, off, 64), __shfl_xor(bh.z, off, 64)));
+                    cl = vmin(cl, mk(__shfl_xor(cl.x, off, 64), __shfl_xor(cl.y, off, 64), __shfl_xor(cl.z, off, 64)));
+                    ch = vmax(ch, mk(__shfl_xor(ch.x, off, 64), __shfl_xor(ch.y, off, 64), __shfl_xor(ch.z, off, 64)));
+                    em = fmaxf(em, __shfl_xor(em, off, 64));
+                }
+                cl = mk(wt_first(cl.x), wt_first(cl.y), wt_first(cl.z));
+                ch = mk(wt_first(ch.x), wt_first(ch.y), wt_first(ch.z));
+                fin = __all(fin);
+                if (lane == 0) {
+                    st_nbox(w.nbox, id, bl, bh);
+                    w.edge[id] = em;
+                }
+                const float cmin[3] = {cl.x, cl.y, cl.z}, cmax[3] = {ch.x, ch.y, ch.z};
+                float sc[3];
+                bool axis_ok[3];
+#pragma unroll
+                for (int x = 0; x < 3; x++) {
+                    axis_ok[x] = cmax[x] > cmin[x];
+                    sc[x] = axis_ok[x] ? (float)WT_NB / (cmax[x] - cmin[x]) : 0.f;
+                }
+                uint32_t nl = m / 2;
+                int best = -1;
+                if (m > 2 && fin && level < WT_DEPTH && (axis_ok[0] || axis_ok[1] || axis_ok[2])) {
+                    uint32_t* bins = &s_bin[wave][0][0][0];
+                    for (uint32_t q = lane; q < 3 * WT_NB; q += 64) {
+                        uint32_t* b = bins + 7 * q;
+                        b[0] = b[1] = b[2] = 0xFFFFFFFFu;
+                        b[3] = b[4] = b[5] = b[6] = 0u;
+                    }
+                    wt_wave_sync();
+                    for (uint32_t p = pa + lane; p <= pb; p += 64) {
+                        const uint32_t j = s_perm[0][p];
+                        uint32_t o[6];
+#pragma unroll
+                        for (int q = 0; q < 6; q++) o[q] = wt_ord(s_box[q][j]);
+#pragma unroll
+                        for (int x = 0; x < 3; x++) {
+                            if (!axis_ok[x]) continue;
+                            uint32_t* b = &s_bin[wave][x][wt_bin(s_box[x][j], s_box[3 + x][j], cmin[x], sc[x])][0];
+                            atomicMin(&b[0], o[0]); atomicMin(&b[1], o[1]); atomicMin(&b[2], o[2]);
+                            atomicMax(&b[3], o[3]); atomicMax(&b[4], o[4]); atomicMax(&b[5], o[5]);
+                            atomicAdd(&b[6], 1u);
+                        }
+                    }
+                    wt_wave_sync();
+                    float cost = INFINITY;
+                    uint32_t cnt_l = 0;
+                    const int x = (int)lane / (WT_NB - 1), plane = (int)lane % (WT_NB - 1);
+                    if (x == 0 ? axis_ok[0] : x == 1 ? axis_ok[1] : x == 2 ? axis_ok[2] : false) {
+                        uint32_t L[6] = {~0u, ~0u, ~0u, 0u, 0u, 0u}, R[6] = {~0u, ~0u, ~0u, 0u, 0u, 0u}, nL = 0, nR = 0;
+#pragma unroll
+                        for (int k = 0; k < WT_NB; k++) {
+                            const uint32_t* b = &s_bin[wave][x][k][0];
+                            const bool isl = k <= plane;
+                            nL += isl ? b[6] : 0u;
+                            nR += isl ? 0u : b[6];
+#pragma unroll
+                            for (int q = 0; q < 3; q++) {
+                                L[q] = isl ? min(L[q], b[q]) : L[q];
+                                L[3 + q] = isl ? max(L[3 + q], b[3 + q]) : L[3 + q];
+                                R[q] = isl ? R[q] : min(R[q], b[q]);
+                                R[3 + q] = isl ? R[3 + q] : max(R[3 + q], b[3 + q]);
+                            }
+                        }
+                        if (nL && nR) {
+                            float lb[6], rb[6];
+#pragma unroll
+                            for (int q = 0; q < 6; q++) { lb[q] = wt_unord(L[q]); rb[q] = wt_unord(R[q]); }
+                            const float c = half_area(lb) * (float)nL + half_area(rb) * (float)nR;
+                            if (c < INFINITY) { cost = c; cnt_l = nL; }
+                        }
+                    }
+                    uint32_t pick = cost < INFINITY ? lane : 0xFFFFu;
+#pragma unroll
+                    for (int off = 32; off > 0; off >>= 1) {
+                        const float oc = __shfl_xor(cost, off, 64);
+                        const uint32_t op = __shfl_xor(pick, off, 64);
+                        if (oc < cost || (oc == cost && op < pick)) { cost = oc; pick = op; }
+                    }
+                    if (pick != 0xFFFFu) {
+                        const uint32_t cn = __shfl(cnt_l, (int)pick, 64);
+                        if (level + 1 + wt_clog2(max(cn, m - cn)) <= s_budget) {
+                            best = (int)(pick / (WT_NB - 1)) * WT_NB + (int)(pick % (WT_NB - 1));
+                            nl = cn;
+                        }
+                    }
+                }
+                if (best >= 0) {
+                    const int x = best / WT_NB, plane = best % WT_NB;
+                    uint32_t base_l = pa, base_r = pa + nl;
+                    for (uint32_t p0 = pa; p0 <= pb; p0 += 64) {
+                        const uint32_t p = p0 + lane;
+                        const bool valid = p <= pb;
+                        const uint32_t j = valid ? s_perm[0][p] : 0u;
+                        const float blo = x == 0 ? s_box[0][j] : x == 1 ? s_box[1][j] : s_box[2][j];
+                        const float bhi = x == 0 ? s_box[3][j] : x == 1 ? s_box[4][j] : s_box[5][j];
+                        const float c0 = x == 0 ? cmin[0] : x == 1 ? cmin[1] : cmin[2];
+                        const float s0 = x == 0 ? sc[0] : x == 1 ? sc[1] : sc[2];
+                        const bool left = valid && wt_bin(blo, bhi, c0, s0) <= plane;
+                        const unsigned long long ml = __ballot(left), mr = __ballot(valid && !left);
+                        const unsigned long long below = (1ull << lane) - 1ull;
+                        if (valid) {
+                            const uint32_t dst = left ? base_l + (uint32_t)__popcll(ml & below)
+                                                      : base_r + (uint32_t)__popcll(mr & below);
+                            if (dst <= pb) s_perm[1][dst] = (uint16_t)j;
+                        }
+                        base_l += (uint32_t)__popcll(ml);
+                        base_r += (uint32_t)__popcll(mr);
+                    }
+                    wt_wave_sync();
+                    for (uint32_t p = pa + lane; p <= pb; p += 64) s_perm[0][p] = s_perm[1][p];
+                    wt_wave_sync();
+                }
+                if (lane == 0) {
+                    const uint32_t la = pa, lb = pa + nl - 1, ra = pa + nl, rb = pb;
+                    const uint32_t idl = la == lb ? (LEAF_BIT | (lo + s_perm[0][la])) : lo + lb;
+                    const uint32_t idr = ra == rb ? (LEAF_BIT | (lo + s_perm[0][ra])) : lo + ra;
+                    w.topo[id] = make_uint4(idl, idr, lo + pa, lo + pb);
+                    if (la != lb) {
+                        w.pint[idl] = id << 1;
+                        const uint32_t q = atomicAdd(&s_nseg[nxt], 1u);
+                        if (q < WT_K / 2) { s_seg[nxt][q][0] = la | lb << 16; s_seg[nxt][q][1] = idl; }
+                    }
+                    if (ra != rb) {
+                        w.pint[idr] = (id << 1) | 1u;
+                        const uint32_t q = atomicAdd(&s_nseg[nxt], 1u);
+                        if (q < WT_K / 2) { s_seg[nxt][q][0] = ra | rb << 16; s_seg[nxt][q][1] = idr; }
+                    }
+                }
+            }
+            __syncthreads();
+            if (tid == 0) s_nseg[cur] = 0;
+            __syncthreads();
+        }
+    }
+}
+
+__global__ __launch_bounds__(BLOCK) void k_wt_qnodes(BuildArgs a, const float* __restrict__ edge) {
+    const uint32_t k = blockIdx.x * BLOCK + threadIdx.x;
+    if (k + 1 >= a.T) return;
+    qnode_nbox(a, k, edge[k]);
+}
+
 inline uint32_t blocks_for(size_t n) { return (uint32_t)((n + BLOCK - 1) / BLOCK); }
 
+}
+
+void launch_walk_tree(const BuildArgs& a, const WalkTree& w, hipStream_t s) {
+    if (a.T < 2) return;
+    (void)hipMemsetAsync(w.roots, 0, sizeof(uint32_t), s);
+    hipLaunchKernelGGL(k_wt_select, dim3(blocks_for(a.T - 1)), dim3(BLOCK), 0, s, a, w);
+    hipLaunchKernelGGL(k_wt_rebuild, dim3(min(4096u, blocks_for(a.T))), dim3(WT_BLOCK), 0, s, a, w);
+    BuildArgs q = a;
+    q.topo = w.topo;
+    q.pint = w.pint;
+    q.nbox = w.nbox;
+    q.qnode = w.qnode;
+    q.rec_on = 0;
+    hipLaunchKernelGGL(k_wt_qnodes, dim3(blocks_for(a.T - 1)), dim3(BLOCK), 0, s, q, w.edge);
 }
 
 void launch_bounds(const BuildArgs& a, hipStream_t s) {
diff --git a/raytracebvh_amd/csrc/rtbvh_internal.h b/raytracebvh_amd/csrc/rtbvh_internal.h
--- a/raytracebvh_amd/csrc/rtbvh_internal.h
+++ b/raytracebvh_amd/csrc/rtbvh_internal.h
@@ -92,6 +92,15 @@
 void launch_morton_sort_small(const BuildArgs& a, hipStream_t s);
 void launch_records(const BuildArgs& a, hipStream_t s);
 void launch_nbox(const BuildArgs& a, hipStream_t s);
+struct WalkTree {
+    uint4* topo;
+    uint32_t* pint;
+    float* nbox;
+    float* edge;
+    QNode* qnode;
+    uint32_t* roots;
+};
+void launch_walk_tree(const BuildArgs& a, const WalkTree& w, hipStream_t s);
 void launch_export(const BuildArgs& a, void* out_nodes, hipStream_t s);
 void launch_from_codes(const BuildArgs& a, const float* leaf_boxes, hipStream_t s);
 
@@ -131,6 +140,7 @@
     float* refl_rec;
     float* refr_rec;
     const QNode* qnode;
+    const QNode* qnode_walk;
     uint32_t* pb_list;
 };
 enum class PrimaryKind { LANE_REFERENCE, LANE_NEAREST, PACKET_REFERENCE, PACKET_NEAREST, PACKET_WIDE, BINNED };
diff --git a/raytracebvh_amd/csrc/trace.hip b/raytracebvh_amd/csrc/trace.hip
--- a/raytracebvh_amd/csrc/trace.hip
+++ b/raytracebvh_amd/csrc/trace.hip
@@ -4023,8 +4023,9 @@
     const bool early = RTBVH_EARLY_SHADE && certified && es;
     const uint32_t nshade = early ? (es->P + ESHADE_RAYS - 1) / ESHADE_RAYS : 0u;
     if (early) hipLaunchKernelGGL(k_hit_init, dim3(1024), dim3(BLOCK), 0, s, hitrec, qin_count);
+    const QNode* qn = certified && a.qnode_walk ? a.qnode_walk : a.qnode;
     const auto launch = [&](auto* kernel) {
-        hipLaunchKernelGGL(kernel, dim3(blocks + nshade), dim3(BLOCK), 0, s, a.inner, a.qnode, a.leaf, a.T, qin, qin_count,
+        hipLaunchKernelGGL(kernel, dim3(blocks + nshade), dim3(BLOCK), 0, s, a.inner, qn, a.leaf, a.T, qin, qin_count,
                            perm, hitrec, next, a.counters, a.overflow, wide ? a.stack_limit4b : a.stack_limit, defer,
                            a.topo, a.nb ? a.nbox : nullptr, blocks, a, early ? es->qout : nullptr,
                            early ? es->qout_count : nullptr, early ? (int)es->emit : 0, early ? es->redo : nullptr,
diff --git a/raytracebvh_amd/graphics.py b/raytracebvh_amd/graphics.py
--- a/raytracebvh_amd/graphics.py
+++ b/raytracebvh_amd/graphics.py
@@ -1050,6 +1050,11 @@
         self._check(_L.lib().rtbvh_read_qnodes(self._h, _L.ptr(out), len(out)))
         return out
 
+    def read_walk_qnodes(self) -> np.ndarray:
+        out = np.zeros((max(2 * self.num_tris - 1, 0), 16), np.uint32)
+        self._check(_L.lib().rtbvh_read_walk_qnodes(self._h, _L.ptr(out), len(out)))
+        return out
+
     def read_morton(self) -> np.ndarray:
         out = np.zeros(self.num_tris, np.uint32)
         self._check(_L.lib().rtbvh_read_morton(self._h, _L.ptr(out)))
```

New measurement: 5438 Mrays/s (median of 6 runs). 1.04x the previous value.
